# tingliu/glia

Hardware: AMD Instinct MI355X
Metric: region_merges_per_sec (higher is better)
Workload: dtype u32 labels / f32 image / f64 statistics and features

## Files before the change

### cli/edge_rebuild_check.cpp

```cpp
#include <cstdio>
#include <cstring>
#include <vector>
#include "../glia_amd/csrc/edge_record.hpp"

using namespace glia;

int main() {
  const uint32_t R = 5, R0 = 1;
  struct E { uint32_t u, v, n; double mean; uint32_t r0; bool h0; };
  const std::vector<E> edges = {{0, 1, 7, 0.125, 1, true},  {0, 2, 3, 0.5, 0, true},       {1, 2, 11, 0.33203125, 0, false}, {1, 3, 1, 0.0, 2, true},
                                {2, 3, 40, 0.99609375, 1, false}, {0, 4, 5, 0.25, 3, true}, {2, 4, 9, 0.7421875, 2, true},    {3, 4, 2, 0.00390625, 1, true}};
  std::vector<uint32_t> deg(R, 0), off(R, 0), cur(R, 0);
  for (const E& e : edges) { ++deg[e.u]; ++deg[e.v]; }
  for (uint32_t r = 1; r < R; ++r) off[r] = off[r - 1] + deg[r - 1];
  std::vector<FatEntry> pool(2 * edges.size());
  std::vector<uint32_t> posu(edges.size()), posv(edges.size());
  for (size_t e = 0; e < edges.size(); ++e) {
    const E& g = edges[e];
    const uint32_t pu = cur[g.u]++, pv = cur[g.v]++;
    FatEntry a; a.eid = (uint32_t)e; a.rs = g.v; a.n = g.n; a.pos = pv; a.off = off[g.v]; a.len = deg[g.v]; a.mean = g.mean;
    FatEntry b = a; b.rs = g.u; b.pos = pu; b.off = off[g.u]; b.len = deg[g.u];
    pool[off[g.u] + pu] = a; pool[off[g.v] + pv] = b;
    posu[e] = pu; posv[e] = pv;
  }
  int checked = 0, cats[3] = {0, 0, 0};
  for (uint32_t v = 0; v < R; ++v) {
    for (uint32_t i = 0; i < deg[v]; ++i) {
      const FatEntry& fe = pool[off[v] + i];
      if (fe.eid == kRecNone || !(fe.rs < v)) continue;
      const E& g = edges[fe.eid];
      const uint32_t rs = g.u, r2 = g.v, k = r2 - R0;
      const uint32_t cat = rs < g.r0 ? 0u : (g.h0 ? 1u : 2u);
      const unsigned long long seq = ((unsigned long long)(k + 1u) << 32) | ((unsigned long long)cat << 30) | rs;
      const double first = g.mean, sal = -first;
      unsigned long long mb, sb;
      memcpy(&mb, &first, 8); memcpy(&sb, &sal, 8);
      const uint32_t want[16] = {rs, r2, posu[fe.eid], posv[fe.eid], (uint32_t)mb, (uint32_t)(mb >> 32), g.n, kRecNone,
                                 off[rs], deg[rs], off[r2], deg[r2], (uint32_t)sb, (uint32_t)(sb >> 32), (uint32_t)seq, (uint32_t)(seq >> 32)};
      const EdgeRec got = rebuild_edge_record(fe, i, v, off[v], deg[v], (uint32_t)((seq >> 30) & 3u), R0);
      if (memcmp(&got, want, 64) != 0) {
        const uint32_t* w = reinterpret_cast<const uint32_t*>(&got);
        printf("edge_rebuild_check: edge %u (%u, %u) differs:", fe.eid, rs, r2);
        for (int j = 0; j < 16; ++j) printf(" %08x/%08x", w[j], want[j]);
        printf("\n");
        return 1;
      }
      ++checked; ++cats[cat];
    }
  }
  if (checked != (int)edges.size() || !cats[0] || !cats[1] || !cats[2]) { printf("edge_rebuild_check: %d of %zu edges visited\n", checked, edges.size()); return 1; }
  printf("edge_rebuild_check: %d records rebuilt from list entries agree with the stored form (cat 0/1/2: %d/%d/%d)\n", checked, cats[0], cats[1], cats[2]);
  return 0;
}
```

### glia_amd/csrc/api.cpp

```cpp
#include <algorithm>
#include <atomic>
#include <cmath>
#include <cstdlib>
#include <cstring>
#include <limits>
#include <mutex>
#include <unordered_map>

#include "rmap_order.hpp"
#include "api_types.hpp"

namespace glia {

static thread_local std::string g_err;
void set_error(const std::string& msg) { g_err = msg; }

static const char* const kOptionKeys[] = {"GLIA_HMT_PB_WINDOW", "GLIA_HMT_PB_BATCH", "GLIA_HMT_WINCAP", "GLIA_HMT_REBASE", "GLIA_HMT_HORIZON",
                                          "GLIA_HMT_FORCE_TREE", "GLIA_HMT_HELPERS", "GLIA_HMT_TRACE", "GLIA_HMT_LIBM", "GLIA_HMT_BC_NOCOMMON",
                                          "GLIA_HMT_BC_GENERIC", "GLIA_HMT_DEBUG", "GLIA_HMT_MAXITERS", "GLIA_HMT_MINCAP", "GLIA_HMT_MEDIAN_BATCH", "GLIA_HMT_BCFEAT", "GLIA_HMT_CC"};
static std::mutex g_opt_mu;
static std::unordered_map<std::string, std::string> g_opt;
static bool g_opt_init = false;
static void opt_init_locked() {
  if (g_opt_init) return;
  for (const char* k : kOptionKeys) if (const char* e = getenv(k)) g_opt[k] = e;
  g_opt_init = true;
}
static bool opt_known(const char* key) { for (const char* k : kOptionKeys) if (!strcmp(k, key)) return true; return false; }
bool option(const char* key, std::string* value) {
  std::lock_guard<std::mutex> lock(g_opt_mu);
  opt_init_locked();
  auto it = g_opt.find(key);
  if (it == g_opt.end()) return false;
  if (value) *value = it->second;
  return true;
}
int set_option(const char* key, const char* value) {
  if (!key || !opt_known(key)) { set_error(std::string("set_option: unknown option ") + (key ? key : "(null)")); return GLIA_HMT_ERR_ARG; }
  std::lock_guard<std::mutex> lock(g_opt_mu);
  opt_init_locked();
  if (value) g_opt[key] = value; else g_opt.erase(key);
  return GLIA_HMT_OK;
}

float ceil_f32(double d) {
  if (std::isinf(d) || std::isnan(d)) return (float)d;
  float f = (float)d;
  if ((double)f < d) f = std::nextafterf(f, std::numeric_limits<float>::infinity());
  return f;
}
static float floor_f32(double d) {
  if (std::isinf(d) || std::isnan(d)) return (float)d;
  float f = (float)d;
  if ((double)f > d) f = std::nextafterf(f, -std::numeric_limits<float>::infinity());
  return f;
}
uint32_t next_pow2(uint64_t v) {
  uint64_t p = 1;
  while (p < v) p <<= 1;
  return (uint32_t)std::min<uint64_t>(p, 1ull << 31);
}

HistSpec make_hist_spec(int bins, double lo, double hi) {
  HistSpec h;
  h.bins = bins;
  double interval = (hi - lo) / bins;
  double b = 0.0;
  for (int i = 0; i < GLIA_HMT_MAX_BINS; ++i) {
    if (i < bins) { b = (i == 0) ? interval : b + interval; h.fb[i] = ceil_f32(b); }
    else h.fb[i] = std::numeric_limits<float>::infinity();
  }
  h.lo_f = floor_f32(lo);
  h.hi_f = ceil_f32(hi);
  return h;
}

static LibmSel probe_host_libm() {
  std::vector<double> xs;
  uint64_t s = 0x9E3779B97F4A7C15ull;
  auto next = [&]() { s ^= s << 13; s ^= s >> 7; s ^= s << 17; return s; };
  for (int i = 0; i < 6000; ++i) { const uint64_t n = 1 + next() % 100000, c = 1 + next() % n; xs.push_back((double)c / (double)n); }
  for (int i = 0; i < 3000; ++i) xs.push_back(1.0 + ((double)(int64_t)(next() % 2000001) - 1000000.0) * 1e-7);
  for (int i = 0; i < 3000; ++i) xs.push_back(std::ldexp(1.0 + (double)(next() >> 12) * 0x1p-52, (int)(next() % 120) - 60));
  for (int e = -1074; e < 1024; e += 37) xs.push_back(std::ldexp(1.0, e));
  LibmSel sel = {kLibmDevice, kLibmDevice, kLibmDevice};
  bool l2 = true, ls = true, lf = true, ps = true, pf = true;
  for (double x : xs) {
    volatile double vx = x;
    const double h2 = std::log2(vx), h1 = std::log(vx);
    l2 = l2 && glibc::as_u64(h2) == glibc::as_u64(glibc::log2_sse2(x));
    ls = ls && glibc::as_u64(h1) == glibc::as_u64(glibc::log_sse2(x));
    lf = lf && glibc::as_u64(h1) == glibc::as_u64(glibc::log_fma(x));
  }
  for (int i = 0; i < 12000; ++i) {
    const double x = i < 4000 ? (double)(i + 1) : (double)(1 + next() % (i < 8000 ? (1ull << 24) : (1ull << 40)));
    volatile double vx = x, vy = 1.5;
    const uint64_t h = glibc::as_u64(std::pow(vx, vy));
    ps = ps && h == glibc::as_u64(glibc::pow_sse2(x, 1.5));
    pf = pf && h == glibc::as_u64(glibc::pow_fma(x, 1.5));
  }
  if (l2) sel.log2_variant = kLibmSse2;
  if (lf) sel.log_variant = kLibmFma; else if (ls) sel.log_variant = kLibmSse2;
  if (pf) sel.pow_variant = kLibmFma; else if (ps) sel.pow_variant = kLibmSse2;
  std::string ov;
  if (option("GLIA_HMT_LIBM", &ov)) {
    const char* e = ov.c_str();
    const int v = !strcmp(e, "sse2") ? kLibmSse2 : !strcmp(e, "fma") ? kLibmFma : kLibmDevice;
    sel.log_variant = v; sel.log2_variant = v == kLibmFma ? kLibmSse2 : v; sel.pow_variant = v;
  }
  return sel;
}

}

static std::atomic<int> g_live_contexts{0};

extern "C" {

const char* glia_hmt_last_error(void) { return g_err.c_str(); }
const char* glia_hmt_version(void) { return "glia_hmt 0.1 (gfx950)"; }

int glia_hmt_ctx_create(int device, void* hip_stream, glia_hmt_ctx** out) {
  if (!out) { set_error("ctx_create: out is NULL"); return GLIA_HMT_ERR_ARG; }
  int n = 0;
  GLIA_HIP_TRY(hipGetDeviceCount(&n));
  if (device < 0 || device >= n) { set_error("ctx_create: no such HIP device"); return GLIA_HMT_ERR_ARG; }
  GLIA_HIP_TRY(hipSetDevice(device));
  glia_hmt_ctx* c = new glia_hmt_ctx;
  c->device = device;
  ++g_live_contexts;
  const int rc = [&]() -> int {
    if (hip_stream) c->stream = (hipStream_t)hip_stream;
    else { GLIA_HIP_TRY(hipStreamCreateWithFlags(&c->stream, hipStreamNonBlocking)); c->own_stream = true; }
    GLIA_HIP_TRY(hipMalloc(&c->flags, 256));
    GLIA_HIP_TRY(hipMemsetAsync(c->flags, 0, 256, c->stream));
    GLIA_HIP_TRY(hipEventCreate(&c->ev0));
    GLIA_HIP_TRY(hipEventCreate(&c->ev1));
    return GLIA_HMT_OK;
  }();
  if (rc) { glia_hmt_ctx_destroy(c); return rc; }
  static const LibmSel sel = probe_host_libm();
  c->libm = sel;
  *out = c;
  if (sel.log2_variant == 0 || sel.log_variant == 0 || sel.pow_variant == 0)
    set_error(std::string("warning: the host libm's ") + (sel.log2_variant == 0 ? "log2 " : "") + (sel.log_variant == 0 ? "log " : "") +
              (sel.pow_variant == 0 ? "pow " : "") + "is not reproduced bit for bit by a restatement (glibc 2.35 FMA / non-FMA builds): "
              "the entropy / log / compactness feature columns are within 1 ulp of this host's values, unpinned; equal classifier scores may order differently");
  return GLIA_HMT_OK;
}

int glia_hmt_ctx_libm(const glia_hmt_ctx* c, int* log2_variant, int* log_variant) {
  if (!c) return GLIA_HMT_ERR_ARG;
  if (log2_variant) *log2_variant = c->libm.log2_variant;
  if (log_variant) *log_variant = c->libm.log_variant;
  return GLIA_HMT_OK;
}

int glia_hmt_ctx_libm_status(const glia_hmt_ctx* c) {
  if (!c) return GLIA_HMT_ERR_ARG;
  return (c->libm.log2_variant != 0 && c->libm.log_variant != 0 && c->libm.pow_variant != 0) ? 1 : 0;
}

int glia_hmt_ctx_libm_pow(const glia_hmt_ctx* c, int* pow_variant) {
  if (!c || !pow_variant) return GLIA_HMT_ERR_ARG;
  *pow_variant = c->libm.pow_variant;
  return GLIA_HMT_OK;
}

int glia_hmt_host_libm_probe_pow(int* pow_variant) {
  if (!pow_variant) return GLIA_HMT_ERR_ARG;
  *pow_variant = probe_host_libm().pow_variant;
  return GLIA_HMT_OK;
}

int glia_hmt_host_rmap_ranks(const uint32_t* labels, const int64_t* first_voxel, int64_t n, int mode, uint32_t* rank) {
  if (!labels || !first_voxel || !rank || n < 0 || mode < 0 || mode > 2) { set_error("host_rmap_ranks: invalid argument"); return GLIA_HMT_ERR_ARG; }
  std::vector<uint32_t> lab(labels, labels + n), out;
  std::vector<long long> first(first_voxel, first_voxel + n);
  for (int64_t i = 1; i < n; ++i) if (lab[i] <= lab[i - 1]) { set_error("host_rmap_ranks: labels must be ascending"); return GLIA_HMT_ERR_ARG; }
  rmap_ranks(lab, first, &out, mode);
  std::copy(out.begin(), out.end(), rank);
  return GLIA_HMT_OK;
}

int glia_hmt_host_libm_probe(int* log2_variant, int* log_variant) {
  const LibmSel sel = probe_host_libm();
  if (log2_variant) *log2_variant = sel.log2_variant;
  if (log_variant) *log_variant = sel.log_variant;
  return GLIA_HMT_OK;
}

int glia_hmt_host_libm_eval(int function, int variant, const double* h_in, double* h_out, int64_t n) {
  if (!h_in || !h_out || n < 0 || function < 0 || function > 2 || (variant != kLibmSse2 && variant != kLibmFma)) {
    set_error("host_libm_eval: invalid argument");
    return GLIA_HMT_ERR_ARG;
  }
  for (int64_t i = 0; i < n; ++i) {
    const double x = h_in[i];
    if (function == 2) h_out[i] = !glibc::pow_in_domain(x, 1.5) ? std::pow(x, 1.5) : variant == kLibmFma ? glibc::pow_fma(x, 1.5) : glibc::pow_sse2(x, 1.5);
    else h_out[i] = function == 0 ? glibc::log2_sse2(x) : variant == kLibmFma ? glibc::log_fma(x) : glibc::log_sse2(x);
  }
  return GLIA_HMT_OK;
}

int glia_hmt_libm_eval(glia_hmt_ctx* c, int function, int variant, const double* d_in, double* d_out, int64_t n) {
  if (!c || !d_in || !d_out || n < 0 || function < 0 || function > 2) { set_error("libm_eval: invalid argument"); return GLIA_HMT_ERR_ARG; }
  GLIA_HIP_TRY(hipSetDevice(c->device));
  return launch_libm_eval(function, variant, d_in, d_out, n, c->stream);
}

unsigned long long glia_hmt_release_cached_memory(void) { return (unsigned long long)glia::BlockCache::get().trim(); }
unsigned long long glia_hmt_internal_errors(void) { return glia::internal_errors(); }
int glia_hmt_set_option(const char* key, const char* value) { return glia::set_option(key, value); }
int glia_hmt_check_merge_order(const uint32_t* h_order, int64_t n_merges, int64_t n_regions, int64_t* first_bad) {
  if ((!h_order && n_merges) || n_merges < 0 || n_regions < 0 || n_regions > 0x7FFFFFFFll) { set_error("check_merge_order: invalid argument"); return GLIA_HMT_ERR_ARG; }
  int64_t bad = -1;
  if (glia::merge_order_is_consistent(h_order, n_merges, (uint32_t)n_regions, &bad)) { if (first_bad) *first_bad = -1; return GLIA_HMT_OK; }
  if (first_bad) *first_bad = bad;
  set_error("check_merge_order: merge " + std::to_string(bad) + " joins a region that does not exist (any more) or creates the wrong one");
  return GLIA_HMT_ERR_ARG;
}

void glia_hmt_ctx_destroy(glia_hmt_ctx* c) {
  if (!c) return;
  (void)hipSetDevice(c->device);
  if (c->stream) (void)hipStreamSynchronize(c->stream);
  (void)free_tables(c);
  if (c->flags) (void)hipFree(c->flags);
  if (c->ev0) (void)hipEventDestroy(c->ev0);
  if (c->ev1) (void)hipEventDestroy(c->ev1);
  if (c->own_stream) (void)hipStreamDestroy(c->stream);
  delete c;
  if (--g_live_contexts <= 0) (void)glia::BlockCache::get().trim();
}

int glia_hmt_ctx_sync(glia_hmt_ctx* c) {
  if (!c) return GLIA_HMT_ERR_ARG;
  GLIA_HIP_TRY(hipStreamSynchronize(c->stream));
  return GLIA_HMT_OK;
}

int glia_hmt_ctx_set_table_hint(glia_hmt_ctx* c, int64_t expected_regions, int64_t expected_pairs) {
  if (!c) return GLIA_HMT_ERR_ARG;
  c->hint_rcap = expected_regions > 0 ? next_pow2((uint64_t)expected_regions * 2) : 0;
  c->hint_pcap = expected_pairs > 0 ? next_pow2((uint64_t)expected_pairs * 2) : 0;
  return GLIA_HMT_OK;
}

int glia_hmt_synth(glia_hmt_ctx* c, int dim, const int64_t dims[3], int S, int G, uint64_t seed, int variant,
                   uint32_t* d_labels, float* d_pb) {
  if (!c || !dims || !d_labels || !d_pb || (dim != 2 && dim != 3) || S <= 0 || G <= 0) {
    set_error("synth: invalid argument");
    return GLIA_HMT_ERR_ARG;
  }
  GLIA_HIP_TRY(hipSetDevice(c->device));
  int64_t N = dims[0] * dims[1] * (dim == 3 ? dims[2] : 1);
  OwnedArrays own;
  uint32_t* d_truth = nullptr;
  int rc = own.alloc(&d_truth, (size_t)N);
  if (rc == GLIA_HMT_OK) rc = launch_synth(dim, dims, S, G, seed, variant, d_labels, d_truth, d_pb, c->stream);
  if (rc == GLIA_HMT_OK) GLIA_HIP_TRY(hipStreamSynchronize(c->stream));
  return rc;
}

int glia_hmt_watershed(glia_hmt_ctx* c, int dim, const int64_t dims[3], const float* d_image, double level, uint32_t* d_labels, uint32_t* n_labels,
                       int* sweeps) {
  if (!c || !dims || !d_image || !d_labels || (dim != 2 && dim != 3) || !(level >= 0.0)) { set_error("watershed: invalid argument"); return GLIA_HMT_ERR_ARG; }
  GLIA_HIP_TRY(hipSetDevice(c->device));
  return watershed_labels(dim, dims, d_image, level, d_labels, n_labels, sweeps, c->stream);
}

int glia_hmt_label_components(glia_hmt_ctx* c, int dim, const int64_t dims[3], const uint32_t* d_labels_in, const uint32_t* d_mask, int mode,
                              uint32_t* d_labels_out, uint32_t* n_components) {
  auto bad = [](const char* what) { set_error(std::string("label_components: ") + what); return GLIA_HMT_ERR_ARG; };
  if (!c || !dims || !d_labels_in || !d_labels_out || !n_components) return bad("ctx, dims, the two volumes and n_components must not be NULL");
  if (dim != 2 && dim != 3) return bad("dim must be 2 or 3");
  const uint64_t most = 0xFFFFFFFEull;
  uint64_t n = 1;
  for (int i = 0; i < dim; ++i) {
    if (dims[i] <= 0) return bad("extents must be positive");
    if ((uint64_t)dims[i] > most / n) return bad("between 1 and 2^32 - 2 voxels");
    n *= (uint64_t)dims[i];
  }
  if (mode < GLIA_HMT_CC_IDENTITY || mode > GLIA_HMT_CC_BINARY_INVERTED) return bad("mode must be 0 (identity), 1 (binary) or 2 (binary, inverted)");
  if (d_labels_out == d_labels_in) return bad("the volume cannot be labelled in place");
  int route = GLIA_HMT_CC_ROUTE_TILED;
  std::string v;
  if (option("GLIA_HMT_CC", &v) && v != "tiled") {
    if (v != "global") return bad(("GLIA_HMT_CC must be tiled or global, not '" + v + "'").c_str());
    route = GLIA_HMT_CC_ROUTE_GLOBAL;
  }
  GLIA_HIP_TRY(hipSetDevice(c->device));
  return label_components(dim, dims, d_labels_in, d_mask, mode, route, d_labels_out, n_components, c->stream);
}

static int overlap_args(const char* who, const glia_hmt_ctx* c, const uint32_t* d_a, const uint32_t* d_b, int64_t n_voxels) {
  auto bad = [&](const char* what) { set_error(std::string(who) + ": " + what); return GLIA_HMT_ERR_ARG; };
  if (!c) return bad("ctx must not be NULL");
  if (!d_a || !d_b) return bad("the two label volumes must not be NULL");
  if (n_voxels < 1 || (uint64_t)n_voxels > 0xFFFFFFFEull) return bad("between 1 and 2^32 - 2 voxels");
  return GLIA_HMT_OK;
}

int glia_hmt_label_overlap(glia_hmt_ctx* c, const uint32_t* d_a, const uint32_t* d_b, const uint32_t* d_mask, int64_t n_voxels, int flags,
                           glia_hmt_overlap_entry* h_entries, int64_t capacity, int64_t* n_entries) {
  auto bad = [](const char* what) { set_error(std::string("label_overlap: ") + what); return GLIA_HMT_ERR_ARG; };
  if (int rc = overlap_args("label_overlap", c, d_a, d_b, n_voxels)) return rc;
  if (!n_entries) return bad("n_entries must not be NULL");
  if (capacity < 0 || (capacity > 0 && !h_entries)) return bad("h_entries must hold `capacity` >= 0 entries");
  if (flags & ~(GLIA_HMT_OVERLAP_DROP_ZERO_A | GLIA_HMT_OVERLAP_DROP_ZERO_B)) return bad("unknown flag bits");
  GLIA_HIP_TRY(hipSetDevice(c->device));
  std::vector<glia_hmt_overlap_entry> table;
  OverlapPass pass;
  if (int rc = label_overlap(d_a, d_b, d_mask, (unsigned long long)n_voxels, flags, c->stream, &table, &pass)) return rc;
  c->evt = glia_hmt_eval_timing{pass.ms, (int64_t)table.size(), pass.repeats};
  *n_entries = (int64_t)table.size();
  if ((int64_t)table.size() > capacity) { set_error("label_overlap: " + std::to_string(table.size()) + " entries, capacity " + std::to_string(capacity)); return GLIA_HMT_ERR_CAPACITY; }
  std::copy(table.begin(), table.end(), h_entries);
  return GLIA_HMT_OK;
}

int glia_hmt_eval(glia_hmt_ctx* c, int n_images, const uint32_t* const* d_res, const uint32_t* const* d_ref, const uint32_t* const* d_mask,
                  const int64_t* n_voxels, int vi_mode, glia_hmt_eval_result* out) {
  auto bad = [](const char* what) { set_error(std::string("eval: ") + what); return GLIA_HMT_ERR_ARG; };
  if (!c) return bad("ctx must not be NULL");
  if (n_images < 1) return bad("at least one image pair");
  if (!d_res || !d_ref || !n_voxels || !out) return bad("d_res, d_ref, n_voxels and out must not be NULL");
  if (vi_mode != GLIA_HMT_VI_REFERENCE && vi_mode != GLIA_HMT_VI_EXACT) return bad("vi_mode must be GLIA_HMT_VI_REFERENCE or GLIA_HMT_VI_EXACT");
  for (int i = 0; i < n_images; ++i) if (int rc = overlap_args("eval", c, d_res[i], d_ref[i], n_voxels[i])) return rc;
  GLIA_HIP_TRY(hipSetDevice(c->device));
  std::vector<std::vector<glia_hmt_overlap_entry>> tables((size_t)n_images);
  std::vector<const glia_hmt_overlap_entry*> ptr((size_t)n_images);
  std::vector<int64_t> len((size_t)n_images);
  glia_hmt_eval_timing t = {0, 0, 0};
  for (int i = 0; i < n_images; ++i) {
    OverlapPass pass;
    if (int rc = label_overlap(d_res[i], d_ref[i], d_mask ? d_mask[i] : nullptr, (unsigned long long)n_voxels[i], GLIA_HMT_OVERLAP_DROP_ZERO_B, c->stream,
                               &tables[i], &pass)) return rc;
    t.ms_count += pass.ms; t.entries += (int64_t)tables[i].size(); t.repeats += pass.repeats;
    ptr[i] = tables[i].data(); len[i] = (int64_t)tables[i].size();
  }
  c->evt = t;
  return overlap_scores(ptr.data(), len.data(), n_images, vi_mode, out);
}

int glia_hmt_last_eval_timing(const glia_hmt_ctx* c, glia_hmt_eval_timing* out) {
  if (!c || !out) { set_error("last_eval_timing: invalid argument"); return GLIA_HMT_ERR_ARG; }
  *out = c->evt;
  return GLIA_HMT_OK;
}

int64_t glia_hmt_transform_keys(const uint32_t* h_order, int64_t n_merges, uint32_t* h_src, uint32_t* h_dst, int64_t capacity) {
  if (!h_order || !h_src || !h_dst || n_merges < 0) { set_error("transform_keys: invalid argument"); return GLIA_HMT_ERR_ARG; }
  std::vector<uint32_t> s, d;
  int rc = transform_keys(h_order, n_merges, &s, &d);
  if (rc) return rc;
  if ((int64_t)s.size() > capacity) { set_error("transform_keys: output capacity too small"); return GLIA_HMT_ERR_CAPACITY; }
  std::copy(s.begin(), s.end(), h_src);
  std::copy(d.begin(), d.end(), h_dst);
  return (int64_t)s.size();
}

int glia_hmt_transform_image(glia_hmt_ctx* c, uint32_t* d_labels, int64_t n_voxels, const uint32_t* h_src, const uint32_t* h_dst,
                             int64_t n_map, const uint32_t* d_mask, int fill_missing) {
  if (!c || !d_labels || n_voxels < 0 || n_map < 0 || (n_map && (!h_src || !h_dst))) { set_error("transform_image: invalid argument"); return GLIA_HMT_ERR_ARG; }
  GLIA_HIP_TRY(hipSetDevice(c->device));
  return transform_image(d_labels, n_voxels, h_src, h_dst, n_map, d_mask, fill_missing, c->stream, &c->transform_ms);
}

int glia_hmt_relabel_image(glia_hmt_ctx* c, uint32_t* d_labels, int64_t n_voxels, int64_t min_size, uint32_t* n_labels) {
  if (!c || !d_labels || n_voxels < 0 || !n_labels) { set_error("relabel_image: invalid argument"); return GLIA_HMT_ERR_ARG; }
  GLIA_HIP_TRY(hipSetDevice(c->device));
  return relabel_image(d_labels, n_voxels, min_size, n_labels, c->stream);
}

double glia_hmt_last_transform_ms(const glia_hmt_ctx* c) { return c ? c->transform_ms : 0.0; }

int64_t glia_hmt_gen_tree(const uint32_t* h_order, int64_t n_merges, uint32_t* node_label, int32_t* parent, int32_t* child0,
                          int32_t* child1, int64_t capacity) {
  if (!h_order || !node_label || !parent || !child0 || !child1 || n_merges < 0) { set_error("gen_tree: invalid argument"); return GLIA_HMT_ERR_ARG; }
  return gen_tree(h_order, n_merges, node_label, parent, child0, child1, capacity);
}

}
```

### glia_amd/csrc/edge_record.hpp

```cpp
#pragma once
#include <stdint.h>

#if defined(__HIPCC__)
#define GLIA_REC_HD __host__ __device__
#else
#define GLIA_REC_HD
#endif

namespace glia {

#if defined(__HIPCC__)
typedef uint2 RecPair;
#else
struct RecPair { uint32_t x, y; };
#endif
constexpr uint32_t kRecNone = 0xFFFFFFFFu;

struct __attribute__((aligned(16))) FatEntry {
  uint32_t eid;
  uint32_t rs;
  uint32_t n;
  uint32_t pos;
  uint32_t off;
  uint32_t len;
  double mean;
};
static_assert(sizeof(FatEntry) == 32, "FatEntry layout");

struct __attribute__((aligned(16))) EdgeRec {
  uint32_t u, v, posu, posv;
  double mean; int n; uint32_t next;
  RecPair hu, hv;
  double sal; unsigned long long seq;
};
static_assert(sizeof(EdgeRec) == 64, "EdgeRec layout");

GLIA_REC_HD inline EdgeRec rebuild_edge_record(const FatEntry& fe, uint32_t idx, uint32_t v, uint32_t voff, uint32_t vlen, uint32_t cat, uint32_t R0) {
  EdgeRec r;
  r.u = fe.rs; r.v = v; r.posu = fe.pos; r.posv = idx;
  r.mean = fe.mean; r.n = (int)fe.n; r.next = kRecNone;
  r.hu.x = fe.off; r.hu.y = fe.len; r.hv.x = voff; r.hv.y = vlen;
  r.sal = -fe.mean;
  r.seq = ((unsigned long long)(v - R0 + 1u) << 32) | ((unsigned long long)(cat & 3u) << 30) | fe.rs;
  return r;
}

}
```

### glia_amd/csrc/greedy.hip

```cpp
#include <atomic>
#include <cstring>
#include <vector>
#include <limits>
#include <rocprim/device/device_scan.hpp>
#include <rocprim/device/device_radix_sort.hpp>
#include <rocprim/device/device_segmented_radix_sort.hpp>

#include "greedy_batch.hpp"

namespace glia {

__global__ void pq_build_level_kernel(PqTree t, int l) {
  const int lane = threadIdx.x & 63;
  uint32_t j = (blockIdx.x * blockDim.x + threadIdx.x) >> 6;
  if (j < t.lv[l].size) (void)pq_recompute_node(t, l, j, lane, true);
}

int pq_setup(DeviceBuffers& buf, PqTree& t, hipStream_t stream) {
  t.nlevels = 0;
  uint32_t n = t.nleaves;
  while (true) {
    n = (n + kFan - 1) / kFan;
    if (t.nlevels >= kMaxLevels) { set_error("greedy: edge table too large"); return GLIA_HMT_ERR_ARG; }
    PqLevel& L = t.lv[t.nlevels++];
    L.size = n;
    int rc;
    if ((rc = buf.get(&L.sal, n, false, stream))) return rc;
    if ((rc = buf.get(&L.seq, n, false, stream))) return rc;
    if ((rc = buf.get(&L.arg, n, false, stream))) return rc;
    if ((rc = buf.get(&L.dirty, n, true, stream))) return rc;
    if (n <= kTopMax) break;
  }
  {
    int rc;
    if ((rc = buf.get(&t.glist[0], t.lv[0].size, false, stream))) return rc;
    if ((rc = buf.get(&t.glist[1], t.lv[0].size, false, stream))) return rc;
    if ((rc = buf.get(&t.gcount, 2, true, stream))) return rc;
  }
  for (int l = 0; l < t.nlevels; ++l) {
    unsigned long long threads = (unsigned long long)t.lv[l].size * 64ull;
    hipLaunchKernelGGL(pq_build_level_kernel, dim3((unsigned)((threads + 255) / 256)), dim3(256), 0, stream, t, l);
  }
  GLIA_HIP_TRY(hipGetLastError());
  return GLIA_HMT_OK;
}

namespace {

__global__ void win_range_kernel(const double* sal, uint32_t E0, unsigned long long* mm) {
  unsigned long long lo = ~0ull, hi = 0ull;
  for (uint32_t i = blockIdx.x * blockDim.x + threadIdx.x; i < E0; i += gridDim.x * blockDim.x) {
    const unsigned long long b = f64_ord(sal[i]);
    lo = b < lo ? b : lo; hi = b > hi ? b : hi;
  }
  atomicMin(&mm[0], lo); atomicMax(&mm[1], hi);
}
__global__ void win_params_kernel(const unsigned long long* mm, uint32_t B, double* range) {
  const double smin = f64_unord(mm[0]), smax = f64_unord(mm[1]);
  range[0] = smin;
  range[1] = smax > smin ? (double)B / (smax - smin) : 0.0;
}
__global__ void win_collect_kernel(const EdgeRec* er, uint32_t n_edges, const uint8_t* rdead, unsigned long long* kseq, uint32_t* vals, uint32_t* counter) {
  const uint32_t e = blockIdx.x * blockDim.x + threadIdx.x;
  if (e >= n_edges) return;
  const unsigned long long q = er[e].seq;
  if (q == 0) return;
  const uint2 uv = *reinterpret_cast<const uint2*>(&er[e].u);
  if (rdead[uv.x] | rdead[uv.y]) return;
  const uint32_t i = atomicAdd(counter, 1u);
  kseq[i] = q; vals[i] = e;
}
__global__ void win_collect_lists_kernel(WinState st, uint32_t n_regions, unsigned long long* kseq, uint32_t* vals, uint32_t cap, uint32_t* counter) {
  const uint32_t r = (blockIdx.x * blockDim.x + threadIdx.x) >> 6, lane = threadIdx.x & 63u;
  if (r >= n_regions || st.rdead[r]) return;
  const uint32_t off = st.adj_off[r], len = st.adj_len[r];
  const double smin = st.wrange[0], scale = st.wrange[1];
  uint32_t rebuilt = 0;
  for (uint32_t base = 0; base < len; base += 64u) {
    const uint32_t i = base + lane;
    unsigned long long q = 0;
    uint32_t e = kNone;
    if (i < len) {
      const FatEntry fe = st.fpool[off + i];
      if (fe.eid != kNone && fe.rs < r && !st.rdead[fe.rs]) {
        e = fe.eid;
        if ((unsigned long long)e >= st.ne_base && win_cell(-fe.mean, smin, scale, st.wB) < st.wch) {
          const EdgeRec rec = rebuild_edge_record(fe, i, r, off, len, st.ecat[e], st.R0);
          st.er[e] = rec;
          q = rec.seq; ++rebuilt;
        } else q = st.er[e].seq;
      }
    }
    const unsigned long long m = __ballot(q != 0);
    if (m == 0) continue;
    const int first = (int)__builtin_ctzll(m);
    uint32_t b0 = 0;
    if ((int)lane == first) b0 = atomicAdd(&counter[0], (uint32_t)__popcll(m));
    b0 = (uint32_t)__shfl((int)b0, first);
    const uint32_t o = b0 + (uint32_t)__popcll(m & ((1ull << lane) - 1ull));
    if (q != 0 && o < cap) { kseq[o] = q; vals[o] = e; }
  }
  if (rebuilt) atomicAdd(&counter[1], rebuilt);
}
__global__ void win_salkey_kernel(const EdgeRec* er, const uint32_t* vals, uint32_t n, unsigned long long* ksal) {
  const uint32_t i = blockIdx.x * blockDim.x + threadIdx.x;
  if (i < n) ksal[i] = f64_ord(er[vals[i]].sal);
}
__global__ void win_baseline_fill_kernel(WinState st, uint32_t n, uint32_t* isort_w, unsigned long long* isort_seq) {
  const uint32_t i = blockIdx.x * blockDim.x + threadIdx.x;
  if (i >= n) return;
  const EdgeRec r = st.er[isort_w[i]];
  isort_seq[i] = r.seq;
  atomicAdd(&st.wcnt[win_cell(r.sal, st.wrange[0], st.wrange[1], st.wB)], 1u);
}
__global__ void win_segments_kernel(WinState st, const uint32_t* isort, uint32_t n, uint32_t* ige) {
  const uint32_t c = blockIdx.x * blockDim.x + threadIdx.x;
  if (c > st.wB) return;
  uint32_t lo = 0, hi = n;
  while (lo < hi) {
    const uint32_t mid = (lo + hi) >> 1;
    if (win_cell(st.er[isort[mid]].sal, st.wrange[0], st.wrange[1], st.wB) >= c) lo = mid + 1; else hi = mid;
  }
  ige[c] = c == 0 ? n : lo;
}
__global__ void adj_fill_fat(GreedyState g, WinState st, uint32_t E0, uint32_t* cursor) {
  const uint32_t e = blockIdx.x * blockDim.x + threadIdx.x;
  if (e >= E0) return;
  const uint32_t u = g.e_u[e], v = g.e_v[e];
  const uint32_t pu = atomicAdd(&cursor[u], 1u), pv = atomicAdd(&cursor[v], 1u);
  const uint32_t ou = g.adj_off[u], ov = g.adj_off[v], lu = g.adj_len[u], lv = g.adj_len[v];
  FatEntry a; a.eid = e; a.rs = v; a.n = (uint32_t)g.e_n[e]; a.pos = pv; a.off = ov; a.len = lv; a.mean = g.e_mean[e];
  FatEntry b = a; b.rs = u; b.pos = pu; b.off = ou; b.len = lu;
  st.fpool[ou + pu] = a; g.e_posu[e] = pu;
  st.fpool[ov + pv] = b; g.e_posv[e] = pv;
  EdgeRec r; r.u = u; r.v = v; r.posu = pu; r.posv = pv; r.mean = g.e_mean[e]; r.n = g.e_n[e]; r.next = kNone;
  r.hu = make_uint2(ou, lu); r.hv = make_uint2(ov, lv); r.sal = g.pq.leaf_sal[e]; r.seq = g.pq.leaf_seq[e];
  st.er[e] = r;
}
__global__ void fat_to_thin(const FatEntry* f, uint2* out, unsigned long long n) {
  const unsigned long long i = (unsigned long long)blockIdx.x * blockDim.x + threadIdx.x;
  if (i < n) { const FatEntry fe = f[i]; out[i] = make_uint2(fe.eid, fe.eid == kNone ? 0u : fe.rs); }
}
__global__ void edge_unpack(GreedyState g, const EdgeRec* er, const uint8_t* rdead, uint32_t n) {
  const uint32_t e = blockIdx.x * blockDim.x + threadIdx.x;
  if (e >= n) return;
  const EdgeRec r = er[e];
  g.e_u[e] = r.u; g.e_v[e] = r.v; g.e_posu[e] = r.posu; g.e_posv[e] = r.posv; g.e_mean[e] = r.mean; g.e_n[e] = r.n;
  g.pq.leaf_sal[e] = r.sal; g.pq.leaf_seq[e] = (rdead[r.u] | rdead[r.v]) ? 0ull : r.seq;
}

__global__ void edge_unpack_live(GreedyState g, const EdgeRec* er, const uint32_t* vals, uint32_t n) {
  const uint32_t i = blockIdx.x * blockDim.x + threadIdx.x;
  if (i >= n) return;
  const uint32_t e = vals[i];
  const EdgeRec r = er[e];
  g.e_u[e] = r.u; g.e_v[e] = r.v; g.e_posu[e] = r.posu; g.e_posv[e] = r.posv; g.e_mean[e] = r.mean; g.e_n[e] = r.n;
  g.pq.leaf_sal[e] = r.sal; g.pq.leaf_seq[e] = r.seq;
}

__global__ void edge_flags(const uint32_t* pa, const uint32_t* pb, long long P, uint32_t* flag, long long* partner) {
  long long i = (long long)blockIdx.x * blockDim.x + threadIdx.x;
  if (i >= P) return;
  uint32_t a = pa[i], b = pb[i];
  long long j = (a < b) ? find_pair(pa, pb, P, b, a) : -1;
  flag[i] = j >= 0 ? 1u : 0u;
  partner[i] = j;
}

__global__ void edge_fill(const uint32_t* pa, const uint32_t* pb, const uint32_t* prec, long long P,
                          const uint32_t* flag, const uint32_t* eidx, const long long* partner,
                          const uint32_t* rlabel, uint32_t R, GreedyState st, uint32_t* deg) {
  long long i = (long long)blockIdx.x * blockDim.x + threadIdx.x;
  if (i >= P || !flag[i]) return;
  const uint32_t e = eidx[i];
  const long long j = partner[i];
  const uint32_t u = find_label(rlabel, R, pa[i]), v = find_label(rlabel, R, pb[i]);
  const uint32_t* wi = &prec[(size_t)i * kPairWords];
  const uint32_t* wj = &prec[(size_t)j * kPairWords];
  double si, sj;
  memcpy(&si, &wi[P_SUM], 8);
  memcpy(&sj, &wj[P_SUM], 8);
  const int n = (int)(wi[P_CNT] + wj[P_CNT]);
  const double mean = sdivide(si + sj, (double)n, 0.0);
  st.e_u[e] = u; st.e_v[e] = v; st.e_mean[e] = mean; st.e_n[e] = n;
  st.pq.leaf_sal[e] = -mean; st.pq.leaf_seq[e] = (unsigned long long)e + 1ull;
  atomicAdd(&deg[u], 1u);
  atomicAdd(&deg[v], 1u);
}

__global__ void adj_fill(GreedyState st, uint32_t E0, uint32_t* cursor) {
  uint32_t e = blockIdx.x * blockDim.x + threadIdx.x;
  if (e >= E0) return;
  const uint32_t u = st.e_u[e], v = st.e_v[e];
  const uint32_t pu = atomicAdd(&cursor[u], 1u), pv = atomicAdd(&cursor[v], 1u);
  st.pool[st.adj_off[u] + pu] = make_uint2(e, v); st.e_posu[e] = pu;
  st.pool[st.adj_off[v] + pv] = make_uint2(e, u); st.e_posv[e] = pv;
}

__global__ void region_sizes(const uint32_t* rrec, uint32_t R, unsigned long long* rsz, double* rsum) {
  uint32_t r = blockIdx.x * blockDim.x + threadIdx.x;
  if (r >= R) return;
  const uint32_t* w = &rrec[(size_t)r * kRegionWords];
  rsz[r] = w[R_CNT];
  double d; memcpy(&d, &w[R_SUM], 8); rsum[r] = d;
}

__global__ void median_collect(VolumeRef vol, const uint32_t* pa, const uint32_t* pb, long long P, const uint32_t* flag,
                               const uint32_t* eidx, const unsigned long long* e_off, uint32_t* cursor, float* out) {
  const long long N = vol.nx * vol.ny * vol.nz;
  const long long p = (long long)blockIdx.x * blockDim.x + threadIdx.x;
  if (p >= N) return;
  const long long x = p % vol.nx, y = (p / vol.nx) % vol.ny, z = p / (vol.nx * vol.ny);
  const uint32_t t = vol.lab[p];
  if (t == kMaskedLabel) return;
  uint32_t nb = t;
  const long long sy = vol.nx, sz = vol.nx * vol.ny;
  const uint32_t* L = vol.lab_nb;
  do {
    uint32_t q;
    if (x > 0 && (q = L[p - 1]) != t && q != kMaskedLabel) { nb = q; break; }
    if (x + 1 < vol.nx && (q = L[p + 1]) != t && q != kMaskedLabel) { nb = q; break; }
    if (y > 0 && (q = L[p - sy]) != t && q != kMaskedLabel) { nb = q; break; }
    if (y + 1 < vol.ny && (q = L[p + sy]) != t && q != kMaskedLabel) { nb = q; break; }
    if (vol.dim == 3) {
      if (z > 0 && (q = L[p - sz]) != t && q != kMaskedLabel) { nb = q; break; }
      if (z + 1 < vol.nz && (q = L[p + sz]) != t && q != kMaskedLabel) { nb = q; break; }
    }
  } while (false);
  if (nb == t) return;
  const long long i = find_pair(pa, pb, P, t < nb ? t : nb, t < nb ? nb : t);
  if (i < 0 || !flag[i]) return;
  const uint32_t e = eidx[i];
  out[e_off[e] + atomicAdd(&cursor[e], 1u)] = vol.pb[p];
}

__global__ void median_from_runs(const unsigned long long* pv_off, const float* pv, unsigned long long nV, const uint32_t* pa, const uint32_t* pb, long long P,
                                 const uint32_t* flag, const uint32_t* eidx, const unsigned long long* e_off, float* out) {
  const unsigned long long v = (unsigned long long)blockIdx.x * blockDim.x + threadIdx.x;
  if (v >= nV) return;
  long long lo = 0, hi = P;
  while (lo < hi) { const long long mid = (lo + hi) >> 1; if (pv_off[mid + 1] <= v) lo = mid + 1; else hi = mid; }
  const long long i = lo;
  const uint32_t a = pa[i], b = pb[i];
  const long long owner = a < b ? i : find_pair(pa, pb, P, b, a);
  if (owner < 0 || !flag[owner]) return;
  const unsigned long long first = owner == i ? 0ull : pv_off[owner + 1] - pv_off[owner];
  out[e_off[eidx[owner]] + first + (v - pv_off[i])] = pv[v];
}

__global__ void median_init(GreedyState st, uint32_t E0) {
  const uint32_t e = blockIdx.x * blockDim.x + threadIdx.x;
  if (e >= E0) return;
  const uint32_t n = (uint32_t)st.e_n[e];
  const double med = (double)st.vals[st.e_off[e] + n / 2u];
  st.e_mean[e] = med;
  st.pq.leaf_sal[e] = st.size_weight ? -med * (double)min(st.rsz[st.e_u[e]], st.rsz[st.e_v[e]]) : -med;
  atomicAdd(&st.rbv[st.e_u[e]], (unsigned long long)n);
  atomicAdd(&st.rbv[st.e_v[e]], (unsigned long long)n);
}

__global__ void fill_leaves_dead(PqTree t, uint32_t from) {
  uint32_t i = from + blockIdx.x * blockDim.x + threadIdx.x;
  if (i < t.nleaves) { t.leaf_seq[i] = 0; t.leaf_sal[i] = -__builtin_inf(); }
}

}

struct WinBaseline {
  unsigned long long *kseq = nullptr, *kseq2 = nullptr, *ksal = nullptr, *ksal2 = nullptr, *iseq = nullptr;
  uint32_t *vals = nullptr, *vals2 = nullptr, *isort = nullptr, *ige = nullptr, *counter = nullptr;
  void* tmp = nullptr; size_t tmp_bytes = 0;
  uint32_t E0 = 0;
  double h_range[2] = {0.0, 0.0};
  long long prev_top_cell = -1;
  unsigned long long prev_ne = 0;
  double horizon_factor = 0.0;
  bool from_lists = false;
  unsigned long long rebuilt_last = 0;

  int init(DeviceBuffers& buf, WinState& ws, const double* leaf_sal, uint32_t n_initial, uint32_t B, uint32_t R, hipStream_t stream) {
    int rc;
    E0 = n_initial;
    unsigned long long* mm; double* range;
    if ((rc = buf.get(&ws.rdead, 2 * (size_t)R, true, stream))) return rc;
    if ((rc = buf.get(&ws.whead, B, false, stream))) return rc;
    if ((rc = buf.get(&ws.wcnt, B, true, stream))) return rc;
    if ((rc = buf.get(&isort, E0, false, stream))) return rc;
    if ((rc = buf.get(&iseq, E0, false, stream))) return rc;
    if ((rc = buf.get(&ige, (size_t)B + 1, false, stream))) return rc;
    if ((rc = buf.get(&mm, 2, false, stream))) return rc;
    if ((rc = buf.get(&range, 2, false, stream))) return rc;
    if ((rc = buf.get(&kseq, E0, false, stream))) return rc;
    if ((rc = buf.get(&kseq2, E0, false, stream))) return rc;
    if ((rc = buf.get(&ksal, E0, false, stream))) return rc;
    if ((rc = buf.get(&ksal2, E0, false, stream))) return rc;
    if ((rc = buf.get(&vals, E0, false, stream))) return rc;
    if ((rc = buf.get(&vals2, E0, false, stream))) return rc;
    if ((rc = buf.get(&counter, 2, true, stream))) return rc;
    GLIA_HIP_TRY(rocprim::radix_sort_pairs_desc(nullptr, tmp_bytes, kseq, kseq2, vals, vals2, (size_t)E0, 0, 64, stream));
    if ((rc = buf.get((char**)&tmp, tmp_bytes ? tmp_bytes : 16, false, stream))) return rc;
    ws.wrange = range; ws.isort = isort; ws.isort_seq = iseq; ws.ige = ige;
    const unsigned long long mm0[2] = {~0ull, 0ull};
    GLIA_HIP_TRY(hipMemcpyAsync(mm, mm0, sizeof(mm0), hipMemcpyHostToDevice, stream));
    hipLaunchKernelGGL(win_range_kernel, dim3(256), dim3(256), 0, stream, leaf_sal, E0, mm);
    hipLaunchKernelGGL(win_params_kernel, dim3(1), dim3(1), 0, stream, mm, B, range);
    GLIA_HIP_TRY(hipGetLastError());
    GLIA_HIP_TRY(hipMemcpyAsync(h_range, range, sizeof(h_range), hipMemcpyDeviceToHost, stream));
    GLIA_HIP_TRY(hipStreamSynchronize(stream));
    return GLIA_HMT_OK;
  }
  int collect(const WinState& ws, uint32_t n_edges, uint32_t n_regions, hipStream_t stream, uint32_t* n_out) {
    GLIA_HIP_TRY(hipMemsetAsync(counter, 0, 2 * sizeof(uint32_t), stream));
    if (from_lists) hipLaunchKernelGGL(win_collect_lists_kernel, dim3((unsigned)(((unsigned long long)n_regions * 64ull + 255ull) / 256ull)), dim3(256), 0, stream, ws, n_regions, kseq, vals, E0, counter);
    else hipLaunchKernelGGL(win_collect_kernel, dim3((n_edges + 255) / 256), dim3(256), 0, stream, ws.er, n_edges, ws.rdead, kseq, vals, counter);
    GLIA_HIP_TRY(hipGetLastError());
    uint32_t h[2] = {0, 0};
    GLIA_HIP_TRY(hipMemcpyAsync(h, counter, sizeof(h), hipMemcpyDeviceToHost, stream));
    GLIA_HIP_TRY(hipStreamSynchronize(stream));
    if (h[0] > E0) { set_error("greedy: more live edges than initial edges (internal error)"); return GLIA_HMT_ERR_INTERNAL; }
    *n_out = h[0]; rebuilt_last = h[1];
    return GLIA_HMT_OK;
  }
  int rebaseline(WinState& ws, uint32_t n_edges, unsigned long long* ctrl, hipStream_t stream) {
    uint32_t n = 0;
    if (int rc = collect(ws, n_edges, ws.R0 + (uint32_t)ctrl[CTRL_MERGES], stream, &n)) return rc;
    if (n) {
      size_t bytes = tmp_bytes;
      GLIA_HIP_TRY(rocprim::radix_sort_pairs_desc(tmp, bytes, kseq, kseq2, vals, vals2, (size_t)n, 0, 64, stream));
      hipLaunchKernelGGL(win_salkey_kernel, dim3((n + 255) / 256), dim3(256), 0, stream, ws.er, vals2, n, ksal);
      bytes = tmp_bytes;
      GLIA_HIP_TRY(rocprim::radix_sort_pairs_desc(tmp, bytes, ksal, ksal2, vals2, isort, (size_t)n, 0, 64, stream));
    }
    GLIA_HIP_TRY(hipMemsetAsync(ws.whead, 0xFF, sizeof(uint32_t) * ws.wB, stream));
    GLIA_HIP_TRY(hipMemsetAsync(ws.wcnt, 0, sizeof(uint32_t) * ws.wB, stream));
    if (n) hipLaunchKernelGGL(win_baseline_fill_kernel, dim3((n + 255) / 256), dim3(256), 0, stream, ws, n, isort, iseq);
    hipLaunchKernelGGL(win_segments_kernel, dim3((ws.wB + 1 + 255) / 256), dim3(256), 0, stream, ws, isort, n, ige);
    GLIA_HIP_TRY(hipGetLastError());
    ws.nsort = n;
    std::string renv;
    ws.rebase_after = option("GLIA_HMT_REBASE", &renv) ? strtoull(renv.c_str(), nullptr, 10) : std::max<unsigned long long>(800000ull, (unsigned long long)n / 2ull);
    ws.wch = 0;
    if (horizon_factor > 0.0 && n > 4096) {
      unsigned long long topkey = 0;
      GLIA_HIP_TRY(hipMemcpyAsync(&topkey, ksal2, sizeof(topkey), hipMemcpyDeviceToHost, stream));
      GLIA_HIP_TRY(hipStreamSynchronize(stream));
      const long long top_cell = (long long)win_cell(f64_unord(topkey), h_range[0], h_range[1], ws.wB);
      if (prev_top_cell >= 0 && n_edges > prev_ne) {
        const double d = (double)std::max<long long>(0, prev_top_cell - top_cell);
        const double delta = std::max(horizon_factor * d * (double)ws.rebase_after / (double)(n_edges - prev_ne), (double)ws.wB / 512.0);
        ws.wch = (double)top_cell > delta ? (uint32_t)((double)top_cell - delta) : 0u;
      }
      prev_top_cell = top_cell; prev_ne = n_edges;
    }
    ws.ne_base = n_edges;
    const double inf = std::numeric_limits<double>::infinity();
    ctrl[CTRL_CTHR] = (unsigned long long)(long long)(ws.wB - 1);
    memcpy(&ctrl[CTRL_TSAL], &inf, 8); ctrl[CTRL_TSEQ] = ~0ull; ctrl[CTRL_IPTR] = 0;
    return GLIA_HMT_OK;
  }
};

static int run_pb_loop(const RagArrays& rag, hipStream_t stream, const PbRequest& req, MergeResult* out) {
  const long long P = rag.P;
  const uint32_t R = (uint32_t)rag.R;
  if (R == 0 || P == 0) return GLIA_HMT_OK;
  const VolumeRef* median_of = req.median_of;
  CallEvents<3> ev;
  int rc;
  if ((rc = ev.create())) return rc;
  GLIA_HIP_TRY(hipEventRecord(ev.ev[0], stream));
  DeviceBuffers buf;
  uint32_t* flag; uint32_t* eidx; long long* partner;
  if ((rc = buf.get(&flag, P + 1, true, stream))) return rc;
  if ((rc = buf.get(&eidx, P + 1, false, stream))) return rc;
  if ((rc = buf.get(&partner, P, false, stream))) return rc;
  hipLaunchKernelGGL(edge_flags, dim3((unsigned)((P + 255) / 256)), dim3(256), 0, stream, rag.d_pa, rag.d_pb, P, flag, partner);
  if ((rc = rocprim_run(buf, stream, [&](void* t, size_t& b) {
        return rocprim::exclusive_scan(t, b, flag, eidx, 0u, (size_t)(P + 1), rocprim::plus<uint32_t>(), stream); }))) return rc;
  uint32_t E0 = 0;
  GLIA_HIP_TRY(hipMemcpyAsync(&E0, eidx + P, sizeof(uint32_t), hipMemcpyDeviceToHost, stream));
  GLIA_HIP_TRY(hipStreamSynchronize(stream));
  if (E0 == 0) return GLIA_HMT_OK;

  GreedyState st;
  memset(&st, 0, sizeof(st));
  st.R0 = R;
  const bool mincap = initial_capacities(E0, 18, 36, &st.Ecap, &st.pool_cap);
  if ((rc = buf.get(&st.adj_off, 2 * (size_t)R, true, stream))) return rc;
  if ((rc = buf.get(&st.adj_len, 2 * (size_t)R + 1, true, stream))) return rc;
  std::string o_window, o_batch, o_txt;
  const bool batch_off = option("GLIA_HMT_PB_BATCH", &o_batch) && o_batch[0] == '0';
  bool window = !median_of && !req.size_weight && !(option("GLIA_HMT_PB_WINDOW", &o_window) && o_window[0] == '0');
  WinState ws;
  memset(&ws, 0, sizeof(ws));
  GrowList edges, entries, values;
  if (window) {
    if ((rc = entries.add(buf, &ws.fpool, st.pool_cap, stream))) return rc;
    if ((rc = edges.add(buf, &ws.er, st.Ecap, stream))) return rc;
    if ((rc = edges.add(buf, &ws.ecat, st.Ecap, stream))) return rc;
  }
  else if ((rc = entries.add(buf, &st.pool, st.pool_cap, stream))) return rc;
  if ((rc = edges.add(buf, &st.e_u, st.Ecap, stream)) || (rc = edges.add(buf, &st.e_v, st.Ecap, stream)) ||
      (rc = edges.add(buf, &st.e_posu, st.Ecap, stream)) || (rc = edges.add(buf, &st.e_posv, st.Ecap, stream)) ||
      (rc = edges.add(buf, &st.e_mean, st.Ecap, stream)) || (rc = edges.add(buf, &st.e_n, st.Ecap, stream, true)) ||
      (rc = edges.add(buf, &st.pq.leaf_sal, st.Ecap, stream)) || (rc = edges.add(buf, &st.pq.leaf_seq, st.Ecap, stream)))
    return rc;
  st.pq.nleaves = st.Ecap;
  if ((rc = buf.get(&st.rsz, 2 * (size_t)R, true, stream))) return rc;
  if ((rc = buf.get(&st.rsum, 2 * (size_t)R, true, stream))) return rc;
  st.cond_n = req.cond_n; st.cond_rpb = req.cond_rpb; st.size_weight = req.size_weight ? 1 : 0;
  st.cond_t0 = req.cond_n > 0 ? (unsigned long long)req.cond_sizes[0] : 0; st.cond_t1 = req.cond_n > 1 ? (unsigned long long)req.cond_sizes[1] : 0;
  hipLaunchKernelGGL(region_sizes, dim3((R + 255) / 256), dim3(256), 0, stream, rag.d_rrec, R, st.rsz, st.rsum);
  if ((rc = buf.get(&st.mark0, 2 * (size_t)R, true, stream))) return rc;
  if ((rc = buf.get(&st.mark1, 2 * (size_t)R, true, stream))) return rc;
  if ((rc = buf.get(&st.order, 3 * ((size_t)R + 16), false, stream))) return rc;
  if ((rc = buf.get(&st.sal_out, (size_t)R + 16, false, stream))) return rc;
  if ((rc = buf.get(&st.ctrl, 16, true, stream))) return rc;
  uint32_t* cursor;
  if ((rc = buf.get(&cursor, 2 * (size_t)R, true, stream))) return rc;

  hipLaunchKernelGGL(fill_leaves_dead, dim3((st.Ecap - E0 + 255) / 256), dim3(256), 0, stream, st.pq, E0);
  hipLaunchKernelGGL(edge_fill, dim3((unsigned)((P + 255) / 256)), dim3(256), 0, stream, rag.d_pa, rag.d_pb, rag.d_prec, P,
                     flag, eidx, partner, rag.d_rlabel, R, st, st.adj_len);
  if ((rc = rocprim_run(buf, stream, [&](void* t, size_t& b) {
        return rocprim::exclusive_scan(t, b, st.adj_len, st.adj_off, 0u, (size_t)R, rocprim::plus<uint32_t>(), stream); }))) return rc;
  if (window) hipLaunchKernelGGL(adj_fill_fat, dim3((E0 + 255) / 256), dim3(256), 0, stream, st, ws, E0, cursor);
  else hipLaunchKernelGGL(adj_fill, dim3((E0 + 255) / 256), dim3(256), 0, stream, st, E0, cursor);
  GLIA_HIP_TRY(hipGetLastError());
  unsigned long long n_values = 0;
  if (median_of) {
    if ((rc = edges.add(buf, &st.e_off, st.Ecap, stream))) return rc;
    if ((rc = buf.get(&st.rbv, 2 * (size_t)R, true, stream))) return rc;
    if ((rc = rocprim_run(buf, stream, [&](void* t, size_t& b) {
          return rocprim::exclusive_scan(t, b, st.e_n, st.e_off, 0ull, (size_t)E0 + 1, rocprim::plus<unsigned long long>(), stream); }))) return rc;
    GLIA_HIP_TRY(hipMemcpyAsync(&n_values, st.e_off + E0, sizeof(n_values), hipMemcpyDeviceToHost, stream));
    GLIA_HIP_TRY(hipStreamSynchronize(stream));
    if (n_values >= 0xFFFFFFFFull) { set_error("merge_order_pb: more than 2^32 boundary voxels (median linkage)"); return GLIA_HMT_ERR_ARG; }
    st.vals_cap = mincap ? std::max(n_values, 1ull) : n_values * 4ull + (1ull << 20);
    float* unsorted;
    if ((rc = values.add(buf, &st.vals, (size_t)st.vals_cap, stream))) return rc;
    if ((rc = buf.get(&unsorted, (size_t)n_values, false, stream))) return rc;
    uint32_t* vcursor;
    if ((rc = buf.get(&vcursor, (size_t)E0, true, stream))) return rc;
    if (median_of->lab) {
      const long long N = median_of->nx * median_of->ny * median_of->nz;
      hipLaunchKernelGGL(median_collect, dim3((unsigned)((N + 255) / 256)), dim3(256), 0, stream, *median_of, rag.d_pa, rag.d_pb, P,
                         flag, eidx, st.e_off, vcursor, unsorted);
    } else {
      if (!rag.d_pv_off) { set_error("merge_order_pb: median linkage needs the volume or the map's boundary values"); return GLIA_HMT_ERR_UNSUPPORTED; }
      if (rag.nV) hipLaunchKernelGGL(median_from_runs, dim3((unsigned)((rag.nV + 255) / 256)), dim3(256), 0, stream, rag.d_pv_off, rag.d_pv, rag.nV, rag.d_pa, rag.d_pb,
                                     (long long)P, flag, eidx, st.e_off, unsorted);
    }
    GLIA_HIP_TRY(hipGetLastError());
    if ((rc = rocprim_run(buf, stream, [&](void* t, size_t& b) {
          return rocprim::segmented_radix_sort_keys(t, b, unsorted, st.vals, (unsigned)n_values, (unsigned)E0, st.e_off, st.e_off + 1, 0, 32, stream); }))) return rc;
    hipLaunchKernelGGL(median_init, dim3((E0 + 255) / 256), dim3(256), 0, stream, st, E0);
    GLIA_HIP_TRY(hipGetLastError());
  }
  unsigned long long ctrl[CTRL_WORDS] = {};
  ctrl[CTRL_EDGES] = E0; ctrl[CTRL_ENTRIES] = 2ull * E0; ctrl[CTRL_STATUS] = ST_RUN; ctrl[CTRL_VALUES] = n_values;
  WinBaseline base;
  if (window) {
    uint32_t B = 256;
    while (B < E0 / 4 && B < (1u << 22)) B <<= 1;
    ws.wB = B; ws.R0 = R;
    ws.wcap = kWinCap; ws.wbudget = kWinBudget;
    ws.force_tree = 0;
    if (option("GLIA_HMT_FORCE_TREE", &o_txt)) ws.force_tree = strtoull(o_txt.c_str(), nullptr, 10);
    if (option("GLIA_HMT_WINCAP", &o_txt)) {
      const uint32_t c = (uint32_t)strtoul(o_txt.c_str(), nullptr, 10);
      if (c >= 16 && c <= kWinCap) { ws.wcap = c; ws.wbudget = c / 2; }
    }
    ws.order = st.order; ws.sal_out = st.sal_out; ws.ctrl = st.ctrl; ws.rsz = st.rsz; ws.rsum = st.rsum;
    ws.mark0 = st.mark0; ws.mark1 = st.mark1; ws.adj_off = st.adj_off; ws.adj_len = st.adj_len;
    ws.pool_cap = st.pool_cap; ws.Ecap = st.Ecap;
    ws.cond_n = st.cond_n; ws.cond_t0 = st.cond_t0; ws.cond_t1 = st.cond_t1; ws.cond_rpb = st.cond_rpb;
    if ((rc = base.init(buf, ws, st.pq.leaf_sal, E0, B, R, stream))) return rc;
    if (req.cond_n <= 0 && !batch_off) base.horizon_factor = option("GLIA_HMT_HORIZON", &o_txt) ? atof(o_txt.c_str()) : 0.5;
    base.from_lists = req.cond_n <= 0 && !batch_off;
    if ((rc = base.rebaseline(ws, E0, ctrl, stream))) return rc;
  } else if ((rc = pq_setup(buf, st.pq, stream))) return rc;
  GLIA_HIP_TRY(hipMemcpyAsync(st.ctrl, ctrl, sizeof(ctrl), hipMemcpyHostToDevice, stream));
  GLIA_HIP_TRY(hipEventRecord(ev.ev[1], stream));


  st.max_iters = window ? 1ull << 22 : 1ull << 16;
  const bool trace = option("GLIA_HMT_TRACE");
  if (option("GLIA_HMT_MAXITERS", &o_txt)) st.max_iters = std::max(1ull, strtoull(o_txt.c_str(), nullptr, 10));
  const auto kernel = [&]() { return !window ? "tree" : req.cond_n > 0 ? "window" : "batch"; };
  const auto unhandled = [&]() {
    set_error(std::string("greedy: the ") + kernel() + " kernel stopped with status " + std::to_string(ctrl[CTRL_STATUS]) + ", which its driver does not handle (internal error)");
    return GLIA_HMT_ERR_INTERNAL;
  };
  while (true) {
    if (window) {
      ws.max_iters = st.max_iters;
      if (req.cond_n > 0) hipLaunchKernelGGL(greedy_window_kernel<true>, dim3(1), dim3(kGreedyThreads), 0, stream, ws);
      else if (batch_off) hipLaunchKernelGGL(greedy_window_kernel<false>, dim3(1), dim3(kGreedyThreads), 0, stream, ws);
      else hipLaunchKernelGGL(greedy_batch_kernel, dim3(1), dim3(kGreedyThreads), 0, stream, ws);
    } else if (median_of) hipLaunchKernelGGL(greedy_pb_kernel<true>, dim3(1), dim3(kGreedyThreads), 0, stream, st);
    else hipLaunchKernelGGL(greedy_pb_kernel<false>, dim3(1), dim3(kGreedyThreads), 0, stream, st);
    GLIA_HIP_TRY(hipGetLastError());
    GLIA_HIP_TRY(hipMemcpyAsync(ctrl, st.ctrl, sizeof(ctrl), hipMemcpyDeviceToHost, stream));
    GLIA_HIP_TRY(hipStreamSynchronize(stream));
    if (trace) fprintf(stderr, "[trace] merge loop launch ended: status %llu, merges %llu of %u regions, edges %llu, list entries %llu, records rebuilt %llu\n", ctrl[CTRL_STATUS], ctrl[CTRL_MERGES], R, ctrl[CTRL_EDGES], ctrl[CTRL_ENTRIES], base.rebuilt_last);
    base.rebuilt_last = 0;
    if (ctrl[CTRL_STATUS] == ST_DONE) break;
    switch (ctrl[CTRL_STATUS]) {
      case ST_RUN:
        if (!window) continue;
        break;
      case ST_REBASE:
        if (!window) return unhandled();
        break;
      case ST_BAD_SALIENCY: set_error("Error: invalid boundary saliency..."); return GLIA_HMT_ERR_SALIENCY;
      case ST_INTERNAL: {
        char msg[256];
        snprintf(msg, sizeof(msg), "greedy: window queue overflow or more merges than regions (internal error: merges %llu of %u regions, %llu edges of %u initial, "
                 "window %llu%s, %s kernel)", ctrl[CTRL_MERGES], R, ctrl[CTRL_EDGES], E0, ctrl[CTRL_WFILL], ctrl[CTRL_WERR] ? " overflowed" : "", kernel());
        set_error(msg);
        return GLIA_HMT_ERR_INTERNAL;
      }
      case ST_NEED_TREE:
        if (!window) return unhandled();
        entries.remove(&ws.fpool);
        edges.remove(&ws.er);
        edges.remove(&ws.ecat);
        if ((rc = entries.add(buf, &st.pool, st.pool_cap, stream))) return rc;
        hipLaunchKernelGGL(fat_to_thin, dim3((unsigned)((ctrl[CTRL_ENTRIES] + 255) / 256)), dim3(256), 0, stream, ws.fpool, st.pool, ctrl[CTRL_ENTRIES]);
        if (base.from_lists) {
          uint32_t n_live = 0;
          if ((rc = base.collect(ws, (uint32_t)ctrl[CTRL_EDGES], R + (uint32_t)ctrl[CTRL_MERGES], stream, &n_live))) return rc;
          hipLaunchKernelGGL(fill_leaves_dead, dim3((st.Ecap + 255) / 256), dim3(256), 0, stream, st.pq, 0u);
          if (n_live) hipLaunchKernelGGL(edge_unpack_live, dim3((n_live + 255) / 256), dim3(256), 0, stream, st, ws.er, base.vals, n_live);
        } else
        hipLaunchKernelGGL(edge_unpack, dim3((unsigned)((ctrl[CTRL_EDGES] + 255) / 256)), dim3(256), 0, stream, st, ws.er, ws.rdead, (uint32_t)ctrl[CTRL_EDGES]);
        GLIA_HIP_TRY(hipGetLastError());
        if ((rc = pq_setup(buf, st.pq, stream))) return rc;
        window = false;
        st.max_iters = 1ull << 16;
        break;
      case ST_NEED_POOL: {
        const unsigned long long ncap = st.pool_cap * 2;
        if ((rc = entries.grow(buf, (size_t)st.pool_cap, (size_t)ncap, stream))) return rc;
        st.pool_cap = ncap; ws.pool_cap = ncap;
        break;
      }
      case ST_NEED_VALUES: {
        if (!median_of) return unhandled();
        const unsigned long long ncap = st.vals_cap * 2;
        if ((rc = values.grow(buf, (size_t)ctrl[CTRL_VALUES], (size_t)ncap, stream))) return rc;
        st.vals_cap = ncap;
        break;
      }
      case ST_NEED_EDGES: {
        if (st.Ecap >= kMaxEdgeSlots) { set_error("greedy: more than 2^32 edge slots needed"); return GLIA_HMT_ERR_ARG; }
        const uint32_t ocap = st.Ecap, ncap = (uint32_t)std::min<unsigned long long>(kMaxEdgeSlots, (unsigned long long)ocap * 2ull);
        if ((rc = edges.grow(buf, ocap, ncap, stream))) return rc;
        st.Ecap = ncap; st.pq.nleaves = ncap; ws.Ecap = ncap;
        hipLaunchKernelGGL(fill_leaves_dead, dim3((ncap - ocap + 255) / 256), dim3(256), 0, stream, st.pq, ocap);
        if (!window && (rc = pq_setup(buf, st.pq, stream))) return rc;
        break;
      }
      default: return unhandled();
    }
    if (window) {
      if ((rc = base.rebaseline(ws, (uint32_t)ctrl[CTRL_EDGES], ctrl, stream))) return rc;
      GLIA_HIP_TRY(hipMemcpyAsync(st.ctrl + CTRL_CTHR, ctrl + CTRL_CTHR, 4 * sizeof(unsigned long long), hipMemcpyHostToDevice, stream));
    }
    unsigned long long zero = ST_RUN;
    GLIA_HIP_TRY(hipMemcpyAsync(st.ctrl + CTRL_STATUS, &zero, sizeof(zero), hipMemcpyHostToDevice, stream));
  }
  GLIA_HIP_TRY(hipEventRecord(ev.ev[2], stream));
  GLIA_HIP_TRY(hipEventSynchronize(ev.ev[2]));
  out->ms_table = ev.ms(0, 1); out->ms_loop = ev.ms(1, 2);
  out->n_scored = (int64_t)ctrl[CTRL_EDGES];
  return copy_merges(out, (int64_t)ctrl[CTRL_MERGES], st.order, st.sal_out);
}


static std::atomic<unsigned long long> g_internal_errors{0};
unsigned long long internal_errors() { return g_internal_errors.load(); }
void count_internal_error() { g_internal_errors.fetch_add(1); }
bool merge_order_is_consistent(const uint32_t* o, int64_t n, uint32_t R, int64_t* first_bad) {
  std::vector<uint8_t> gone(2 * (size_t)R + 1, 0);
  for (int64_t k = 0; k < n; ++k) {
    const uint32_t a = o[3 * k], b = o[3 * k + 1], c = o[3 * k + 2];
    if (k >= (int64_t)R || c != R + (uint32_t)k || a >= c || b >= c || a == b || gone[a] || gone[b]) { if (first_bad) *first_bad = k; return false; }
    gone[a] = gone[b] = 1;
  }
  return true;
}
int finish_merge_order(int rc, const uint32_t* o, int64_t n, uint32_t R, hipStream_t stream) {
  int64_t bad = -1;
  if (rc == GLIA_HMT_OK && !merge_order_is_consistent(o, n, R, &bad)) {
    set_error("greedy: merge " + std::to_string(bad) + " of " + std::to_string(n) + " joins a region that does not exist (any more) or creates the wrong one (internal error)");
    rc = GLIA_HMT_ERR_INTERNAL;
  }
  if (rc == GLIA_HMT_ERR_INTERNAL) { count_internal_error(); (void)hipStreamSynchronize(stream); }
  return rc;
}
int greedy_mean(const RagArrays& rag, hipStream_t stream, const PbRequest& req, MergeResult* out) {
  const int rc = run_pb_loop(rag, stream, req, out);
  return finish_merge_order(rc, out->order.data(), out->n, (uint32_t)rag.R, stream);
}

}
```

### glia_amd/csrc/greedy_batch.hpp

```cpp
#pragma once
#include "greedy_window.hpp"

namespace glia {
namespace {

constexpr uint32_t kBatchKill = 32;
constexpr int kMemP = 3;
constexpr uint32_t kMemMax = 192;
struct BatchShared {
  alignas(16) Key part1[kNW];
  alignas(16) Key part2[kNW];
  uint32_t nkill, kovf; alignas(16) uint32_t kill[kBatchKill];
  uint32_t byrank[kNW];
  uint32_t bitmap[kNW][64];
  uint32_t m_newcount[kNW], m_total[kNW], m_ok[kNW];
  double m_maxsal[kNW];
  uint32_t bad;
};

template <int CTRL, int ROW_MASK = 0xf>
__device__ __forceinline__ void top2_ord_step(unsigned long long& a1, unsigned long long& a2) {
  const unsigned long long b1 = dpp64<CTRL, ROW_MASK, ROW_MASK != 0xf>(a1), b2 = dpp64<CTRL, ROW_MASK, ROW_MASK != 0xf>(a2);
  const bool g = b1 > a1;
  const unsigned long long hi = g ? b1 : a1, lo = g ? a1 : b1, m2 = b2 > a2 ? b2 : a2;
  a1 = hi; a2 = lo > m2 ? lo : m2;
}
__device__ __forceinline__ void wave_top2_ord(unsigned long long& a1, unsigned long long& a2) {
  top2_ord_step<0xB1>(a1, a2);
  top2_ord_step<0x4E>(a1, a2);
  top2_ord_step<0x124>(a1, a2);
  top2_ord_step<0x128>(a1, a2);
  top2_ord_step<0x142, 0xa>(a1, a2);
  top2_ord_step<0x143, 0xc>(a1, a2);
  a1 = lane_u64(a1, 63); a2 = lane_u64(a2, 63);
}

#ifdef GLIA_HMT_PROFILE
__device__ unsigned long long g_scanprof[8];
__device__ unsigned long long g_scanfill[3][3];
#define SCAN_T(i) do { if (tid == 0) { const unsigned long long tn_ = __builtin_readcyclecounter(); g_scanprof[i] += tn_ - st_; st_ = tn_; } } while (0)
#else
#define SCAN_T(i) do {} while (0)
#endif
enum { kScanOther = 0, kScanNarrow = 1, kScanWide = 2 };
__device__ __forceinline__ void batch_scan(const WinState& st, WinShared& w, BatchShared& b, int tid, [[maybe_unused]] int from) {
#ifdef GLIA_HMT_PROFILE
  unsigned long long st_ = __builtin_readcyclecounter();
  if (tid == 0) g_scanprof[7] += 1;
#endif
  const uint32_t n = w.n < st.wcap ? w.n : st.wcap, nk = b.nkill < kBatchKill ? b.nkill : kBatchKill, kovf = b.kovf;
#ifdef GLIA_HMT_PROFILE
  if (tid == 0) g_scanfill[from][n <= 512u ? 0 : n <= 1024u ? 1 : 2] += 1;
#endif
  const uint32_t own = 64u * (uint32_t)(((tid >> 6) + (tid & 63)) & 7) + (uint32_t)(tid & 63);
  Key k1, k2;
  k1.sal = -__builtin_inf(); k1.seq = 0; k1.arg = 0; k2 = k1;
  auto pass = [&](auto nb_tag) {
    constexpr int NB = decltype(nb_tag)::value;
    unsigned long long q[NB]; uint32_t e[NB]; double sl[NB];
#pragma unroll
    for (int j = 0; j < NB; ++j) { const uint32_t i = own + (uint32_t)j * kGreedyThreads; q[j] = w.seq[i]; e[j] = w.e[i]; sl[j] = w.sal[i]; }
    const uint4 ka = *reinterpret_cast<const uint4*>(&b.kill[0]), kb = *reinterpret_cast<const uint4*>(&b.kill[4]);
    const uint32_t kl[8] = {ka.x, ka.y, ka.z, ka.w, kb.x, kb.y, kb.z, kb.w};
    SCAN_T(0);
    uint32_t deadm[NB];
#pragma unroll
    for (int j = 0; j < NB; ++j) {
      uint32_t d = 0;
#pragma unroll
      for (uint32_t t = 0; t < 8; ++t) d |= (uint32_t)(t < nk) & (uint32_t)(kl[t] == e[j]);
      deadm[j] = d;
    }
    if (nk > 8u) {
      for (uint32_t t = 8; t < nk; ++t) {
        const uint32_t kt = b.kill[t];
#pragma unroll
        for (int j = 0; j < NB; ++j) deadm[j] |= (uint32_t)(kt == e[j]);
      }
      if (kovf) {
        full_barrier();
#pragma unroll
        for (int j = 0; j < NB; ++j) {
          const uint32_t i = own + (uint32_t)j * kGreedyThreads;
          if (i < n && q[j] != 0) deadm[j] |= (uint32_t)(st.er[e[j]].seq == 0);
        }
      }
    }
#pragma unroll
    for (int j = 0; j < NB; ++j) {
      const uint32_t i = own + (uint32_t)j * kGreedyThreads;
      const bool was = (i < n) & (q[j] != 0);
      const bool live = was & (deadm[j] == 0u);
      if (was & !live) w.seq[i] = 0;
      Key c; c.sal = live ? sl[j] : -__builtin_inf(); c.seq = live ? q[j] : 0ull; c.arg = i;
      const bool b1 = better(c, k1), b2 = better(c, k2);
      k2.sal = b1 ? k1.sal : (b2 ? c.sal : k2.sal); k2.seq = b1 ? k1.seq : (b2 ? c.seq : k2.seq); k2.arg = b1 ? k1.arg : (b2 ? c.arg : k2.arg);
      k1.sal = b1 ? c.sal : k1.sal; k1.seq = b1 ? c.seq : k1.seq; k1.arg = b1 ? c.arg : k1.arg;
    }
  };
  static_assert(kWinPer == 3, "batch_scan: one pass instance per number of blocks");
  const uint32_t nu = (uint32_t)__builtin_amdgcn_readfirstlane((int)n);
  if (nu > 2u * kGreedyThreads) pass(std::integral_constant<int, 3>{});
  else if (nu > kGreedyThreads) pass(std::integral_constant<int, 2>{});
  else pass(std::integral_constant<int, 1>{});
  SCAN_T(1);
  const int lane = tid & 63;
  const unsigned long long o1 = f64_ord(k1.sal), o2 = f64_ord(k2.sal);
  unsigned long long M1 = o1, M2 = o2;
  wave_top2_ord(M1, M2);
  const unsigned long long t1 = __ballot(o1 == M1), t1l = __ballot((o1 == M1) & (k1.seq != 0ull));
  const int l1 = (int)__builtin_ctzll(t1);
  const bool win1 = lane == l1;
  Key kk; kk.sal = win1 ? k2.sal : k1.sal; kk.seq = win1 ? k2.seq : k1.seq; kk.arg = win1 ? k2.arg : k1.arg;
  const unsigned long long oc = win1 ? o2 : o1;
  const unsigned long long t2 = __ballot(oc == M2), t2l = __ballot((oc == M2) & (kk.seq != 0ull));
  Key m1, m2;
  if (__popcll(t1) == 1 || t1l == 0ull) {
    m1 = lane_key(k1, l1);
    int src = (int)__builtin_ctzll(t2);
    if (__popcll(t2) != 1 && t2l != 0ull) {
#ifdef GLIA_HMT_PROFILE
      if (tid == 0) g_scanprof[5] += 1;
#endif
      const unsigned long long ms = wave_max_u64(oc == M2 ? kk.seq : 0ull);
      src = (int)__builtin_ctzll(__ballot((oc == M2) & (kk.seq == ms)));
    }
    m2 = lane_key(kk, src);
    SCAN_T(2);
  } else {
#ifdef GLIA_HMT_PROFILE
    if (tid == 0) g_scanprof[6] += 1;
#endif
    unsigned long long S1 = o1 == M1 ? k1.seq : 0ull, S2 = o2 == M1 ? k2.seq : 0ull;
    wave_top2_ord(S1, S2);
    const int w1 = (int)__builtin_ctzll(__ballot((o1 == M1) & (k1.seq == S1)));
    const bool winr = lane == w1;
    Key kc; kc.sal = winr ? k2.sal : k1.sal; kc.seq = winr ? k2.seq : k1.seq; kc.arg = winr ? k2.arg : k1.arg;
    const unsigned long long occ = winr ? o2 : o1;
    m1 = lane_key(k1, w1);
    m2 = lane_key(kc, (int)__builtin_ctzll(__ballot((occ == M1) & (kc.seq == S2))));
    SCAN_T(3);
  }
  if ((tid & 63) == 0) { b.part1[tid >> 6] = m1; b.part2[tid >> 6] = m2; }
  full_barrier();
  SCAN_T(4);
  if (tid == 0) { b.nkill = 0; b.kovf = 0; }
}

#ifdef GLIA_HMT_PROFILE
__device__ unsigned long long g_wideprof[8];
__device__ unsigned long long g_edgeprof[3][2];
#define WIDE_T(i) do { if (tid == 0) { const unsigned long long tn_ = __builtin_readcyclecounter(); g_wideprof[i] += tn_ - wt_; wt_ = tn_; } } while (0)
#else
#define WIDE_T(i) do {} while (0)
#endif
__device__ __forceinline__ uint32_t batch_contract_wide(const WinState& st, WinShared& w, WinWork& s, BatchShared& b, int tid, uint32_t slot, double rootsal,
                                                      unsigned long long k, unsigned long long ne, unsigned long long pool_used, double smin, double scale, uint32_t* newcount_out) {
  const uint32_t e = w.e[slot], r0 = w.u[slot], r1 = w.v[slot];
  const uint2 h0r = w.hu[slot], h1r = w.hv[slot];
  const uint32_t wn_now = w.n;
  const uint32_t off0 = h0r.x, len0 = h0r.y, off1 = h1r.x, len1 = h1r.y;
  const uint32_t total = len0 + len1;
  const uint32_t r2 = st.R0 + (uint32_t)k;
  const uint32_t r2off = (uint32_t)pool_used;
#ifdef GLIA_HMT_PROFILE
  unsigned long long wt_ = __builtin_readcyclecounter();
#endif
  lds_barrier();
  WIDE_T(0);
  if (tid == 0) {
    w.seq[slot] = 0;
    st.order[3 * k + 0] = r0; st.order[3 * k + 1] = r1; st.order[3 * k + 2] = r2;
    st.sal_out[k] = rootsal;
    st.er[e].seq = 0;
    st.rdead[r0] = 1; st.rdead[r1] = 1;
  }
  const bool small = total <= kMarkMax;
  win_stage_lists(st, s, tid, e, off0, len0, off1, len1, small);
  if (small) lds_barrier(); else full_barrier();
  WIDE_T(1);
  if (wn_now + total > st.wcap && wn_now > st.wcap / 2u) win_compact(w, tid, st.wcap);
  WIDE_T(2);
  const WinTau tau = {w.cthr, w.tsal, w.tseq, smin, scale};
  const uint32_t nwork = small ? s.nitems : total;
  const uint32_t lenR2 = small ? nwork : 0u;
  bool bad = false;
  uint32_t pend_e = kNone, pend_old = kNone;
#ifdef GLIA_HMT_PROFILE
  uint32_t ep_above = 0, ep_below = 0;
#endif
  auto rounds = [&](auto small_tag) {
    constexpr bool SMALL = decltype(small_tag)::value;
    for (uint32_t base = 0; base < nwork; base += kGreedyThreads) {
      const uint32_t i = base + tid;
      if (i >= nwork) break;
      FatEntry f0, f1;
      bool h0, h1;
      uint32_t rs;
      if (!win_match<SMALL>(st, s, i, e, off0, len0, off1, &rs, &h0, &h1, &f0, &f1)) continue;
      const uint32_t idx = atomicAdd(&s.newcount, 1u);
      const uint32_t newE = (uint32_t)ne + idx;
      double first;
      int second;
      if (mean_link(h0, f0.mean, (int)f0.n, h1, f1.mean, (int)f1.n, &first, &second)) bad = true;
      const uint32_t offRs = f0.off, posRs = f0.pos, lenRs = f0.len;
      if (h0 && h1) st.fpool[offRs + f1.pos].eid = kNone;
      const unsigned long long seq = update_seq(k, rs, r0, h0);
      const double sal = -first;
      const uint32_t cell = win_cell(sal, tau.smin, tau.scale, st.wB);
#ifdef GLIA_HMT_PROFILE
      if (cell < st.wch) ++ep_below; else ++ep_above;
#endif
      store_new_edge<true>(st, newE, rs, r2, posRs, idx, first, second, sal, seq, offRs, lenRs, r2off, lenR2, cell);
      win_queue_edge<true>(st, w, tau, newE, sal, seq, rs, r2, make_uint2(offRs, lenRs), make_uint2(r2off, lenR2), cell, pend_e, pend_old);
      if (h0) win_retire_edge<true, false, kBatchKill>(st, tau, f0.eid, -f0.mean, &b.nkill, b.kill, &b.kovf);
      if (h1) win_retire_edge<true, false, kBatchKill>(st, tau, f1.eid, -f1.mean, &b.nkill, b.kill, &b.kovf);
    }
  };
  if (small) rounds(std::true_type{}); else rounds(std::false_type{});
  if (bad) b.bad = 1;
  WIDE_T(3);
  if (small) lds_barrier(); else full_barrier();
  WIDE_T(4);
  const uint32_t newcount = s.newcount;
  if (!small) win_complete_r2<true>(st, tid, (uint32_t)ne, r2off, newcount, smin, scale);
  if (!small) for (uint32_t i = tid; i < (w.n < st.wcap ? w.n : st.wcap); i += kGreedyThreads) if (w.v[i] == r2) w.hv[i].y = newcount;
  if (pend_e != kNone) st.er[pend_e].next = pend_old;
  if (tid == 0) { st.adj_off[r2] = r2off; st.adj_len[r2] = newcount; }
  lds_barrier();
  WIDE_T(5);
#ifdef GLIA_HMT_PROFILE
  if (ep_above) atomicAdd(&g_edgeprof[small ? 1 : 2][0], (unsigned long long)ep_above);
  if (ep_below) atomicAdd(&g_edgeprof[small ? 1 : 2][1], (unsigned long long)ep_below);
#endif
  if (tid == 0) { s.nitems = 0; s.newcount = 0; }
  *newcount_out = newcount;
  return total;
}

__global__ __launch_bounds__(kGreedyThreads) void greedy_batch_kernel(WinState st) {
  __shared__ WinShared w;
  __shared__ WinWork s;
  __shared__ BatchShared b;
  const int tid = threadIdx.x, lane = tid & 63, wave = tid >> 6;
  unsigned long long k = st.ctrl[CTRL_MERGES], ne = st.ctrl[CTRL_EDGES], pool_used = st.ctrl[CTRL_ENTRIES];
  uint32_t status = ST_RUN;
  win_enter(st, w, s, tid);
  if (tid == 0) { b.nkill = 0; b.kovf = 0; b.bad = 0; }
  b.bitmap[wave][lane] = 0;
  if (tid < kNW) { Key z; z.sal = -__builtin_inf(); z.seq = 0; z.arg = 0; b.part1[tid] = z; b.part2[tid] = z; }
  full_barrier();
  const double smin = st.wrange[0], scale = st.wrange[1];
  uint32_t pend_e = kNone, pend_old = kNone;
  constexpr uint32_t kTab = kMarkSlots / kNW;
  uint32_t* const tk = &s.mk[wave * kTab]; uint32_t* const t0 = &s.mv0[wave * kTab]; uint32_t* const t1 = &s.mv1[wave * kTab];
  static_assert(sizeof(s.stage) >= (size_t)kNW * kTab * 20, "per-wave staging");
  uint32_t* const sg_eid = reinterpret_cast<uint32_t*>(&s.stage[0]) + wave * kTab;
  uint32_t* const sg_n = reinterpret_cast<uint32_t*>(&s.stage[0]) + (kNW + wave) * kTab;
  uint32_t* const sg_pos = reinterpret_cast<uint32_t*>(&s.stage[0]) + (2 * kNW + wave) * kTab;
  double* const sg_mean = reinterpret_cast<double*>(reinterpret_cast<uint32_t*>(&s.stage[0]) + 3 * kNW * kTab) + wave * kTab;
#ifdef GLIA_HMT_PROFILE
  unsigned long long bph[8] = {0, 0, 0, 0, 0, 0, 0, 0}, blast = __builtin_readcyclecounter(), brounds = 0, bmembers = 0, bvalid = 0, bwide = 0, bcut_sal = 0, bcut_dep = 0;
  unsigned long long bw_n[4] = {0, 0, 0, 0}, bw_cyc[4] = {0, 0, 0, 0}, bw_ent[4] = {0, 0, 0, 0}, bw_new[4] = {0, 0, 0, 0};
  uint32_t bep_above = 0, bep_below = 0;
  unsigned long long bsel[2] = {0, 0}, bsel_n[2] = {0, 0};
#define BPH0(wide) do { if (tid == 0) { unsigned long long tn = __builtin_readcyclecounter(); bph[0] += tn - blast; bsel[wide] += tn - blast; bsel_n[wide] += 1; blast = tn; } } while (0)
#define BPH(i) do { if (tid == 0) { unsigned long long tn = __builtin_readcyclecounter(); bph[i] += tn - blast; blast = tn; } } while (0)
#else
#define BPH(i) do {} while (0)
#define BPH0(wide) do {} while (0)
#endif

  for (unsigned long long it = 0; it < st.max_iters; ++it) {
    if (ne - st.ne_base > st.rebase_after) { status = ST_REBASE; break; }
    const int gi = lane >> 3, gj = lane & 7;
    const Key A = b.part1[gi], B = b.part1[gj], C = b.part2[gi];
    const unsigned long long beats = __ballot(better(A, B)), under = __ballot(better(C, B));
    const unsigned long long col = 0x0101010101010101ull << gj;
    const uint32_t rank = (uint32_t)__popcll(beats & col);
    const bool cand_ok = B.seq != 0 && (under & col) == 0;
    if (gi == 0 && cand_ok) b.byrank[rank] = (uint32_t)gj;
    const unsigned long long okmask = __ballot(gi == 0 && cand_ok);
    const uint32_t M = (uint32_t)__popcll(okmask);
    if (M == 0) {
      BPH(5);
      if (pend_e != kNone) { st.er[pend_e].next = pend_old; pend_e = kNone; }
      if (st.force_tree && k >= st.force_tree) { status = ST_NEED_TREE; break; }
      const int r = win_reload(st, w, tid, reinterpret_cast<double*>(&s.stage[0]), reinterpret_cast<unsigned long long*>(&s.stage[0]) + kSelMax);
      BPH(6);
      if (r == 1) { status = ST_DONE; break; }
      if (r == 2) { status = ST_NEED_TREE; break; }
      if (r == 3) { status = ST_REBASE; break; }
      batch_scan(st, w, b, tid, kScanOther);
      continue;
    }
    const unsigned long long minemask = __ballot(gi == 0 && cand_ok && rank == (uint32_t)wave);
    const bool member = minemask != 0;
    const int cj = member ? (int)__builtin_ctzll(minemask) : 0;
    const Key me = b.part1[cj];
    const uint32_t slot = me.arg;
    const uint32_t e = w.e[slot], r0 = w.u[slot], r1 = w.v[slot];
    const uint2 h0r = w.hu[slot], h1r = w.hv[slot];
    const uint32_t off0 = h0r.x, len0 = h0r.y, off1 = h1r.x, len1 = h1r.y;
    const uint32_t total = len0 + len1;
    if (k >= (unsigned long long)st.R0) { status = ST_INTERNAL; break; }
    const unsigned long long firstmask = __ballot(gi == 0 && cand_ok && rank == 0u);
    const Key top = b.part1[__builtin_ctzll(firstmask)];
    const uint2 th0 = w.hu[top.arg], th1 = w.hv[top.arg];
    const uint32_t top_total = th0.y + th1.y;
    BPH0(top_total > kMemMax ? 1 : 0);
    if (top_total > kMemMax) {
      if (ne + top_total > st.Ecap) { status = ST_NEED_EDGES; break; }
      if (pool_used + top_total > st.pool_cap) { status = ST_NEED_POOL; break; }
      uint32_t newcount = 0;
#ifdef GLIA_HMT_PROFILE
      const unsigned long long tw0 = __builtin_readcyclecounter();
#endif
      const uint32_t tt = batch_contract_wide(st, w, s, b, tid, top.arg, top.sal, k, ne, pool_used, smin, scale, &newcount);
      if (b.bad) { status = ST_BAD_SALIENCY; break; }
      k += 1; ne += newcount; pool_used += tt;
#ifdef GLIA_HMT_PROFILE
      bwide += 1;
      { const int cls = tt <= 512u ? 0 : tt <= kMarkMax ? 1 : tt <= 8192u ? 2 : 3; bw_n[cls] += 1; bw_cyc[cls] += __builtin_readcyclecounter() - tw0; bw_ent[cls] += tt; bw_new[cls] += newcount; }
#endif
      batch_scan(st, w, b, tid, kScanWide);
      if (w.spill_ord) { if (pend_e != kNone) { st.er[pend_e].next = pend_old; pend_e = kNone; } win_evict(st, w, tid); batch_scan(st, w, b, tid, kScanOther); }
      BPH(4);
      continue;
    }
    const bool narrow = member && total <= kMemMax;
    b.bitmap[wave][lane] = 0;
    FatEntry fe[kMemP];
    bool act[kMemP], side1[kMemP];
    uint32_t h[kMemP];
#pragma unroll
    for (int p = 0; p < kMemP; ++p) {
      const uint32_t i = (uint32_t)lane + 64u * (uint32_t)p;
      const bool inlist = narrow && i < total;
      side1[p] = i >= len0;
      fe[p].eid = kNone; fe[p].rs = 0; fe[p].n = 0; fe[p].pos = 0; fe[p].off = 0; fe[p].len = 0; fe[p].mean = 0.0;
      if (inlist) fe[p] = st.fpool[side1[p] ? off1 + (i - len0) : off0 + i];
      act[p] = inlist;
    }
    if (pend_e != kNone) { st.er[pend_e].next = pend_old; pend_e = kNone; }
#pragma unroll
    for (int p = 0; p < kMemP; ++p) {
      act[p] = act[p] && fe[p].eid != e && fe[p].eid != kNone;
      h[p] = (fe[p].rs * 2654435761u) >> 24;
      if (act[p]) {
        while (true) {
          const uint32_t old = atomicCAS(&tk[h[p]], 0u, fe[p].rs + 1u);
          if (old == 0u || old == fe[p].rs + 1u) break;
          h[p] = (h[p] + 1u) & (kTab - 1u);
        }
        if (side1[p]) {
          t1[h[p]] = 1u;
          sg_eid[h[p]] = fe[p].eid; sg_n[h[p]] = fe[p].n; sg_pos[h[p]] = fe[p].pos; sg_mean[h[p]] = fe[p].mean;
        } else t0[h[p]] = 1u;
        atomicOr(&b.bitmap[wave][(fe[p].rs >> 5) & 63u], 1u << (fe[p].rs & 31u));
      }
    }
    if (narrow && lane == 0) { atomicOr(&b.bitmap[wave][(r0 >> 5) & 63u], 1u << (r0 & 31u)); atomicOr(&b.bitmap[wave][(r1 >> 5) & 63u], 1u << (r1 & 31u)); }
    asm volatile("s_waitcnt lgkmcnt(0)" ::: "memory");
    bool owner[kMemP], both[kMemP];
    uint32_t p_eid[kMemP], p_n[kMemP], p_pos[kMemP];
    double p_mean[kMemP];
#pragma unroll
    for (int p = 0; p < kMemP; ++p) {
      const uint32_t m0 = act[p] ? t0[h[p]] : 0u, m1 = act[p] ? t1[h[p]] : 0u;
      owner[p] = act[p] && (!side1[p] || m0 == 0u);
      both[p] = owner[p] && !side1[p] && m1 != 0u;
      p_eid[p] = sg_eid[h[p]]; p_n[p] = sg_n[h[p]]; p_pos[p] = sg_pos[h[p]]; p_mean[p] = sg_mean[h[p]];
    }
#pragma unroll
    for (int p = 0; p < kMemP; ++p) if (act[p]) { tk[h[p]] = 0u; t0[h[p]] = 0u; t1[h[p]] = 0u; }
    double first[kMemP]; int second[kMemP]; uint32_t idx[kMemP];
    bool bad = false;
    uint32_t newcount = 0;
    double mx = -__builtin_inf();
#pragma unroll
    for (int p = 0; p < kMemP; ++p) {
      const bool h0 = owner[p] && !side1[p], h1 = owner[p] && (side1[p] || both[p]);
      bad = mean_link(h0, fe[p].mean, (int)fe[p].n, h1, both[p] ? p_mean[p] : fe[p].mean, both[p] ? (int)p_n[p] : (int)fe[p].n, &first[p], &second[p]) || bad;
      const double f = first[p];
      const unsigned long long ownmask = __ballot(owner[p]);
      idx[p] = newcount + (uint32_t)__popcll(ownmask & ((1ull << lane) - 1ull));
      newcount += (uint32_t)__popcll(ownmask);
      mx = (owner[p] && -f > mx) ? -f : mx;
    }
#pragma unroll
    for (int d = 32; d >= 1; d >>= 1) { const double o = __shfl_xor(mx, d); mx = o > mx ? o : mx; }
    if (lane == 0) { b.m_newcount[wave] = narrow ? newcount : 0u; b.m_total[wave] = narrow ? total : 0xFFFFFFFFu; b.m_maxsal[wave] = mx; }
    if (bad) b.bad = 1;
    const uint32_t wn_round = w.n;
    lds_barrier();
    BPH(1);
    if (b.bad) { status = ST_BAD_SALIENCY; break; }
    uint32_t V, ne_off, pool_off, my_ne, my_pool;
    {
      const uint32_t j = (uint32_t)lane & 7u;
      const Key kj = b.part1[b.byrank[j]];
      const uint32_t u = w.u[kj.arg], v = w.v[kj.arg];
      const uint32_t tj = b.m_total[j], nj = b.m_newcount[j];
      double pm = -__builtin_inf();
      uint32_t hit = 0, pre_n = 0, pre_t = 0;
#pragma unroll
      for (uint32_t i = 0; i < (uint32_t)kNW; ++i) {
        const double ms = b.m_maxsal[i];
        const uint32_t bu = b.bitmap[i][(u >> 5) & 63u], bv = b.bitmap[i][(v >> 5) & 63u];
        const uint32_t ti = b.m_total[i], ni = b.m_newcount[i];
        if (i < j) { pm = ms > pm ? ms : pm; hit |= ((bu >> (u & 31u)) | (bv >> (v & 31u))) & 1u; pre_n += ni; pre_t += ti; }
      }
      const bool okj = j < M && tj != 0xFFFFFFFFu && (j == 0u || (kj.sal > pm && hit == 0u));
      const uint32_t okbits = (uint32_t)(__ballot(lane < kNW && okj) & 0xFFull);
      V = (uint32_t)__builtin_ctz(~okbits);
#ifdef GLIA_HMT_PROFILE
      if (V < M) { const uint32_t cutsal = (uint32_t)(__ballot(lane < kNW && j == V && !(kj.sal > pm)) & 0xFFull); if (cutsal) bcut_sal += 1; else bcut_dep += 1; }
#endif
      my_ne = (uint32_t)__builtin_amdgcn_readlane((int)pre_n, wave); my_pool = (uint32_t)__builtin_amdgcn_readlane((int)pre_t, wave);
      const uint32_t last = V - 1u;
      ne_off = (uint32_t)__shfl((int)(pre_n + nj), (int)last); pool_off = (uint32_t)__shfl((int)(pre_t + tj), (int)last);
    }
    const uint32_t sum_tot = pool_off;
    if (ne + sum_tot > st.Ecap) { status = ST_NEED_EDGES; break; }
    if (pool_used + sum_tot > st.pool_cap) { status = ST_NEED_POOL; break; }
    bool popped = false;
    if (wn_round + ne_off > st.wcap && wn_round > st.wcap / 2u) {
      if ((uint32_t)wave < V && lane == 0) w.seq[slot] = 0;
      popped = true;
      lds_barrier();
      win_compact(w, tid, st.wcap);
    }
    const WinTau tau = {w.cthr, w.tsal, w.tseq, smin, scale};
    BPH(2);
    if ((uint32_t)wave < V) {
      const unsigned long long kk = k + (unsigned long long)wave;
      const uint32_t r2 = st.R0 + (uint32_t)kk;
      const uint32_t r2off = (uint32_t)pool_used + my_pool;
      if (lane == 0) {
        if (!popped) w.seq[slot] = 0;
        st.order[3 * kk + 0] = r0; st.order[3 * kk + 1] = r1; st.order[3 * kk + 2] = r2;
        st.sal_out[kk] = me.sal;
        st.er[e].seq = 0;
        st.rdead[r0] = 1; st.rdead[r1] = 1;
        st.adj_off[r2] = r2off; st.adj_len[r2] = newcount;
      }
#pragma unroll
      for (int p = 0; p < kMemP; ++p) {
        if (!owner[p]) continue;
        const bool h0 = !side1[p];
        const uint32_t rs = fe[p].rs;
        const uint32_t newE = (uint32_t)ne + my_ne + idx[p];
        const uint32_t offRs = fe[p].off, posRs = fe[p].pos, lenRs = fe[p].len;
        if (both[p]) st.fpool[offRs + p_pos[p]].eid = kNone;
        const unsigned long long seq = update_seq(kk, rs, r0, h0);
        const double sal = -first[p];
        const uint32_t cell = win_cell(sal, tau.smin, tau.scale, st.wB);
#ifdef GLIA_HMT_PROFILE
        if (cell < st.wch) ++bep_below; else ++bep_above;
#endif
        store_new_edge<true>(st, newE, rs, r2, posRs, idx[p], first[p], second[p], sal, seq, offRs, lenRs, r2off, newcount, cell);
        win_queue_edge<true>(st, w, tau, newE, sal, seq, rs, r2, make_uint2(offRs, lenRs), make_uint2(r2off, newcount), cell, pend_e, pend_old);
        win_retire_edge<true, false, kBatchKill>(st, tau, fe[p].eid, -fe[p].mean, &b.nkill, b.kill, &b.kovf);
        if (both[p]) win_retire_edge<true, false, kBatchKill>(st, tau, p_eid[p], -p_mean[p], &b.nkill, b.kill, &b.kovf);
      }
    }
    lds_barrier();
    BPH(3);
#ifdef GLIA_HMT_PROFILE
    brounds += 1; bmembers += M; bvalid += V;
#endif
    k += V; ne += ne_off; pool_used += pool_off;
    batch_scan(st, w, b, tid, kScanNarrow);
    if (w.spill_ord) { if (pend_e != kNone) { st.er[pend_e].next = pend_old; pend_e = kNone; } win_evict(st, w, tid); batch_scan(st, w, b, tid, kScanOther); }
    BPH(4);
  }
#ifdef GLIA_HMT_PROFILE
  if (bep_above) atomicAdd(&g_edgeprof[0][0], (unsigned long long)bep_above);
  if (bep_below) atomicAdd(&g_edgeprof[0][1], (unsigned long long)bep_below);
  full_barrier();
  if (tid == 0) printf("[batch profile] created edges at or above / below the horizon (cumulative): narrow commit %llu / %llu  wide on the LDS table %llu / %llu  wide on the global marks %llu / %llu\n",
                       atomicAdd(&g_edgeprof[0][0], 0ull), atomicAdd(&g_edgeprof[0][1], 0ull), atomicAdd(&g_edgeprof[1][0], 0ull), atomicAdd(&g_edgeprof[1][1], 0ull),
                       atomicAdd(&g_edgeprof[2][0], 0ull), atomicAdd(&g_edgeprof[2][1], 0ull));
  if (tid == 0) printf("[batch profile] merges %llu: select %llu  compute %llu  validate %llu  commit %llu  scan %llu  loop-top %llu  reload %llu (cycles); rounds %llu candidates %llu committed %llu (cut by saliency %llu, by adjacency %llu) wide %llu\n",
                       k, bph[0], bph[1], bph[2], bph[3], bph[4], bph[5], bph[6], brounds, bmembers, bvalid, bcut_sal, bcut_dep, bwide);
  if (tid == 0) printf("[batch profile] scan phases (cumulative cycles, wave 0): loads %llu  compare %llu  top2 %llu  top2 with a tied best %llu  barrier %llu  calls %llu  tied second %llu  tied best %llu\n",
                       g_scanprof[0], g_scanprof[1], g_scanprof[2], g_scanprof[3], g_scanprof[4], g_scanprof[7], g_scanprof[5], g_scanprof[6]);
  if (tid == 0) printf("[batch profile] scan fill (cumulative; n <= 512, <= 1024, more): after reload/evict %llu %llu %llu  after narrow round %llu %llu %llu  after wide %llu %llu %llu\n",
                       g_scanfill[0][0], g_scanfill[0][1], g_scanfill[0][2], g_scanfill[1][0], g_scanfill[1][1], g_scanfill[1][2], g_scanfill[2][0], g_scanfill[2][1], g_scanfill[2][2]);
  if (tid == 0) printf("[batch profile] loop top (this launch): narrow rounds %llu cycles %llu  wide pops %llu cycles %llu\n", bsel_n[0], bsel[0], bsel_n[1], bsel[1]);
  if (tid == 0) printf("[batch profile] wide phases (cumulative cycles): entry-barrier %llu  lists+table %llu  compact %llu  main loop (wave 0) %llu  loop barrier %llu  tail %llu\n",
                       g_wideprof[0], g_wideprof[1], g_wideprof[2], g_wideprof[3], g_wideprof[4], g_wideprof[5]);
  if (tid == 0) printf("[batch profile] wide by entries (<=512, <=1408, <=8192, more): n %llu %llu %llu %llu  cycles %llu %llu %llu %llu  entries %llu %llu %llu %llu  new edges %llu %llu %llu %llu\n",
                       bw_n[0], bw_n[1], bw_n[2], bw_n[3], bw_cyc[0], bw_cyc[1], bw_cyc[2], bw_cyc[3], bw_ent[0], bw_ent[1], bw_ent[2], bw_ent[3], bw_new[0], bw_new[1], bw_new[2], bw_new[3]);
#endif
  if (pend_e != kNone) st.er[pend_e].next = pend_old;
  full_barrier();
  win_leave(st, w, tid, k, ne, pool_used, status);
}

}
}
```

### glia_amd/csrc/greedy_window.hpp

```cpp
#pragma once
#include "greedy_tree.hpp"
#include "edge_record.hpp"

namespace glia {
namespace {

static_assert(kRecNone == kNone, "edge_record.hpp");
struct WinState {
  EdgeRec* er; FatEntry* fpool;
  uint32_t* whead;
  uint32_t* wcnt;
  const uint32_t* isort; const unsigned long long* isort_seq;
  const uint32_t* ige;
  const double* wrange;
  uint32_t* order; double* sal_out; unsigned long long* ctrl;
  unsigned long long* rsz; double* rsum; uint32_t *mark0, *mark1, *adj_off, *adj_len;
  unsigned long long pool_cap, max_iters, cond_t0, cond_t1;
  double cond_rpb;
  uint32_t R0, Ecap, wB, nsort;
  unsigned long long ne_base, rebase_after;
  uint32_t wcap, wbudget;
  int cond_n;
  uint32_t wch;
  uint8_t* rdead;
  unsigned long long force_tree;
  uint8_t* ecat;
};
constexpr uint32_t kWinCap = 1536;
constexpr uint32_t kWinBudget = 768;
constexpr uint32_t kWinMinLoad = 192;
constexpr uint32_t kWinMinPartial = 96;
constexpr uint32_t kKillMax = 8;
constexpr int kNW = kGreedyThreads / 64;
constexpr int kWinPer = (int)(kWinCap / kGreedyThreads);
static_assert(kWinPer * kGreedyThreads == (int)kWinCap, "window capacity");
struct WinShared {
  double sal[kWinCap];
  unsigned long long seq[kWinCap];
  uint32_t e[kWinCap], u[kWinCap], v[kWinCap];
  uint2 hu[kWinCap], hv[kWinCap];
  int cthr; uint32_t iptr;
  double tsal; unsigned long long tseq;
  alignas(16) uint32_t n;
  uint32_t nk, kovf, pad0;
  alignas(16) uint32_t kill[kKillMax];
  alignas(16) Key part[kNW];
  uint32_t touched[2][64];
  uint32_t wsum[kNW];
  uint32_t bcast, maxcell, err, need_tree;
  double psal; unsigned long long pseq;
  unsigned long long spill_ord;
};
struct WinWork {
  uint32_t mk[kMarkSlots], mv0[kMarkSlots], mv1[kMarkSlots];
  uint32_t items[kMarkMax], newidx[kMarkMax], nitems, newcount, bad;
  FatEntry stage[kMarkMax];
};

__host__ __device__ __forceinline__ uint32_t win_cell(double sal, double smin, double scale, uint32_t B) {
  double t = (sal - smin) * scale;
  t = t > 0.0 ? t : 0.0;
  return t >= (double)(B - 1u) ? B - 1u : (uint32_t)t;
}
__device__ __forceinline__ bool win_above(int cthr, double tsal, unsigned long long tseq, int cell, double sal, unsigned long long seq) {
  return cell > cthr || (cell == cthr && (sal > tsal || (sal == tsal && seq > tseq)));
}

__device__ __forceinline__ uint32_t block_scan_incl(uint32_t v, uint32_t* wsum, int tid, uint32_t* total) {
  const int lane = tid & 63, wave = tid >> 6;
  uint32_t x = v;
#pragma unroll
  for (int d = 1; d < 64; d <<= 1) { const uint32_t y = (uint32_t)__shfl_up((int)x, d); if (lane >= d) x += y; }
  full_barrier();
  if (lane == 63) wsum[wave] = x;
  full_barrier();
  uint32_t base = 0, tot = 0;
#pragma unroll
  for (int i = 0; i < kNW; ++i) { const uint32_t s = wsum[i]; if (i < wave) base += s; tot += s; }
  *total = tot;
  return base + x;
}

__device__ __forceinline__ void win_put(WinShared& w, uint32_t slot, double sal, unsigned long long seq, uint32_t e, uint32_t u, uint32_t v, uint2 hu, uint2 hv) {
  w.sal[slot] = sal; w.seq[slot] = seq; w.e[slot] = e; w.u[slot] = u; w.v[slot] = v; w.hu[slot] = hu; w.hv[slot] = hv;
}
__device__ __forceinline__ void win_take(const WinState& st, WinShared& w, uint32_t e, const EdgeRec& r) {
  if (r.seq != 0) {
    const uint32_t slot = atomicAdd(&w.n, 1u);
    if (slot < st.wcap) win_put(w, slot, r.sal, r.seq, e, r.u, r.v, r.hu, r.hv); else w.err = 1;
  }
}

__device__ __forceinline__ void win_scan(const WinState& st, WinShared& w, int tid, uint32_t r2, uint32_t r2len) {
  const uint4 hd = *reinterpret_cast<const uint4*>(&w.n);
  const uint4 k0 = *reinterpret_cast<const uint4*>(&w.kill[0]), k1 = *reinterpret_cast<const uint4*>(&w.kill[4]);
  unsigned long long q[kWinPer]; uint32_t e[kWinPer], v[kWinPer]; double sl[kWinPer];
#pragma unroll
  for (int j = 0; j < kWinPer; ++j) { const uint32_t i = (uint32_t)tid + (uint32_t)j * kGreedyThreads; q[j] = w.seq[i]; e[j] = w.e[i]; v[j] = w.v[i]; sl[j] = w.sal[i]; }
  const uint32_t n = hd.x, nk = hd.y < kKillMax ? hd.y : kKillMax;
  const uint32_t kl[kKillMax] = {k0.x, k0.y, k0.z, k0.w, k1.x, k1.y, k1.z, k1.w};
  Key k;
  k.sal = -__builtin_inf(); k.seq = 0; k.arg = 0;
#pragma unroll
  for (int j = 0; j < kWinPer; ++j) {
    const uint32_t i = (uint32_t)tid + (uint32_t)j * kGreedyThreads;
    bool live = i < n && q[j] != 0;
    bool dead = false;
    if (nk) {
#pragma unroll
      for (uint32_t t = 0; t < kKillMax; ++t) dead = dead || (t < nk && kl[t] == e[j]);
    }
    if (live && hd.z) dead = dead || st.er[e[j]].seq == 0;
    if (live && dead) { w.seq[i] = 0; live = false; }
    if (live && v[j] == r2) w.hv[i].y = r2len;
    Key c; c.sal = live ? sl[j] : -__builtin_inf(); c.seq = live ? q[j] : 0ull; c.arg = i;
    if (better(c, k)) k = c;
  }
  k = wave_max(k);
  if ((tid & 63) == 0) w.part[tid >> 6] = k;
  lds_barrier();
  if (tid == 0) { w.nk = 0; w.kovf = 0; }
}
__device__ __forceinline__ Key win_root(const WinShared& w, int lane) {
  static_assert(kNW == 8, "win_root");
  Key k = w.part[lane & (kNW - 1)];
  key_max_step<0xB1>(k); key_max_step<0x4E>(k);
  const Key a = lane_key(k, 0), b = lane_key(k, 4);
  return better(b, a) ? b : a;
}

__device__ __forceinline__ uint32_t win_compact(WinShared& w, int tid, uint32_t cap = kWinCap) {
  double sal[kWinPer]; unsigned long long seq[kWinPer]; uint32_t e[kWinPer], u[kWinPer], v[kWinPer]; uint2 hu[kWinPer], hv[kWinPer];
  uint32_t live = 0;
  const uint32_t n = w.n < cap ? w.n : cap;
#pragma unroll
  for (int j = 0; j < kWinPer; ++j) {
    const uint32_t i = (uint32_t)tid * kWinPer + j;
    seq[j] = i < n ? w.seq[i] : 0ull;
    sal[j] = w.sal[i]; e[j] = w.e[i]; u[j] = w.u[i]; v[j] = w.v[i]; hu[j] = w.hu[i]; hv[j] = w.hv[i];
    live += seq[j] != 0;
  }
  uint32_t total;
  uint32_t o = block_scan_incl(live, w.wsum, tid, &total) - live;
#pragma unroll
  for (int j = 0; j < kWinPer; ++j) if (seq[j] != 0) { win_put(w, o, sal[j], seq[j], e[j], u[j], v[j], hu[j], hv[j]); ++o; }
  if (tid == 0) w.n = total;
  full_barrier();
  return total;
}

__device__ __forceinline__ void win_push_global(const WinState& st, uint32_t e, uint32_t cell) {
  const uint32_t old = atomicExch(&st.whead[cell], e);
  st.er[e].next = old;
  atomicAdd(&st.wcnt[cell], 1u);
}

__device__ __forceinline__ void win_flush(const WinState& st, WinShared& w, int tid) {
  const double smin = st.wrange[0], scale = st.wrange[1];
  if (tid == 0) w.maxcell = 0;
  full_barrier();
  const uint32_t n = w.n < st.wcap ? w.n : st.wcap;
  uint32_t mc = 0;
  for (uint32_t i = tid; i < n; i += kGreedyThreads) {
    if (w.seq[i] == 0) continue;
    const uint32_t c = win_cell(w.sal[i], smin, scale, st.wB);
    win_push_global(st, w.e[i], c);
    mc = mc > c + 1u ? mc : c + 1u;
  }
  if (mc) atomicMax(&w.maxcell, mc);
  full_barrier();
  if (tid == 0) {
    if (w.maxcell && (int)w.maxcell - 1 >= w.cthr) { w.cthr = (int)w.maxcell - 1; w.tsal = __builtin_inf(); w.tseq = ~0ull; }
    w.n = 0;
  }
  full_barrier();
}

__device__ __forceinline__ void win_evict(const WinState& st, WinShared& w, int tid) {
  const double smin = st.wrange[0], scale = st.wrange[1];
  const double lim = f64_unord(w.spill_ord);
  const uint32_t n = w.n < st.wcap ? w.n : st.wcap;
  full_barrier();
  for (uint32_t i = tid; i < n; i += kGreedyThreads) {
    if (w.seq[i] == 0 || w.sal[i] > lim) continue;
    win_push_global(st, w.e[i], win_cell(w.sal[i], smin, scale, st.wB));
    w.seq[i] = 0;
  }
  full_barrier();
  if (tid == 0) { w.n = n; w.cthr = (int)win_cell(lim, smin, scale, st.wB); w.tsal = lim; w.tseq = ~0ull; w.spill_ord = 0; }
  full_barrier();
}

__device__ __forceinline__ void win_take_initial(const WinState& st, WinShared& w, uint32_t a, uint32_t b, int tid) {
  for (uint32_t i = a + (uint32_t)tid; i < b; i += kGreedyThreads) { const uint32_t e = st.isort[i]; const EdgeRec r = st.er[e]; win_take(st, w, e, r); }
}

constexpr uint32_t kSelMax = 384;
__device__ __forceinline__ int win_reload(const WinState& st, WinShared& w, int tid, double* sel_sal, unsigned long long* sel_seq) {
  full_barrier();
  if (tid == 0) { w.n = 0; w.need_tree = 0; }
  full_barrier();
  uint32_t c_hi = (uint32_t)(w.cthr + 1) < st.wB ? (uint32_t)(w.cthr + 1) : st.wB, loaded = 0, iptr = w.iptr;
  int result = 1;
  const uint32_t c_floor = st.wch < st.wB ? st.wch : 0u;
  while (c_hi > c_floor) {
    const bool valid = (uint32_t)tid < c_hi - c_floor;
    const uint32_t c = valid ? c_hi - 1u - (uint32_t)tid : 0u;
    const uint32_t cn = valid ? ld_relaxed(&st.wcnt[c]) : 0u;
    uint32_t total;
    const uint32_t incl = block_scan_incl(cn, w.wsum, tid, &total);
    const bool ok = valid && incl <= st.wbudget - loaded;
    const uint32_t m = (uint32_t)__syncthreads_count(ok ? 1 : 0);
    const uint32_t nvalid = c_hi - c_floor < (uint32_t)kGreedyThreads ? c_hi - c_floor : (uint32_t)kGreedyThreads;
    if (m != 0) {
      const uint32_t c_lo = c_hi - m;
      if ((uint32_t)tid == m - 1u) w.bcast = incl;
      const uint32_t i_to = st.ige[c_lo];
      win_take_initial(st, w, iptr, i_to, tid);
      iptr = i_to > iptr ? i_to : iptr;
      if ((uint32_t)tid < m) {
        uint32_t e = ld_relaxed(&st.whead[c]);
        if (e != kNone) {
          st_agent(&st.whead[c], kNone);
          if (cn != 0) while (e != kNone) { const EdgeRec r = st.er[e]; win_take(st, w, e, r); e = r.next; }
        }
        if (cn != 0) st_agent(&st.wcnt[c], 0u);
      }
      full_barrier();
      loaded += w.bcast;
      c_hi = c_lo;
      if (loaded) result = 0;
    }
    if (m < nvalid) {
      const uint32_t room = st.wbudget - loaded;
      const uint32_t cs = c_hi - 1u;
      if (room >= (kWinMinPartial < st.wbudget / 8u ? kWinMinPartial : st.wbudget / 8u) || loaded == 0) {
        const uint32_t K = (room / 2u < kSelMax ? room / 2u : kSelMax) > 1u ? (room / 2u < kSelMax ? room / 2u : kSelMax) : 2u, RA = room > K ? room - K : 1u;
        const uint32_t seg_end = st.ige[cs];
        const uint32_t before = w.n;
        if (tid == 0) {
          uint32_t hn = 0, nlive = 0;
          for (uint32_t e = ld_relaxed(&st.whead[cs]); e != kNone;) {
            const EdgeRec r = st.er[e];
            if (r.seq != 0) {
              ++nlive;
              if (hn < K) {
                uint32_t i = hn++;
                while (i > 0) {
                  const uint32_t p = (i - 1u) >> 1;
                  if (!(sel_sal[p] > r.sal || (sel_sal[p] == r.sal && sel_seq[p] > r.seq))) break;
                  sel_sal[i] = sel_sal[p]; sel_seq[i] = sel_seq[p]; i = p;
                }
                sel_sal[i] = r.sal; sel_seq[i] = r.seq;
              } else if (r.sal > sel_sal[0] || (r.sal == sel_sal[0] && r.seq > sel_seq[0])) {
                uint32_t i = 0;
                while (true) {
                  uint32_t c = 2u * i + 1u;
                  if (c >= hn) break;
                  if (c + 1u < hn && (sel_sal[c + 1u] < sel_sal[c] || (sel_sal[c + 1u] == sel_sal[c] && sel_seq[c + 1u] < sel_seq[c]))) ++c;
                  if (!(sel_sal[c] < r.sal || (sel_sal[c] == r.sal && sel_seq[c] < r.seq))) break;
                  sel_sal[i] = sel_sal[c]; sel_seq[i] = sel_seq[c]; i = c;
                }
                sel_sal[i] = r.sal; sel_seq[i] = r.seq;
              }
            }
            e = r.next;
          }
          w.psal = nlive > K ? sel_sal[0] : -__builtin_inf(); w.pseq = nlive > K ? sel_seq[0] : 0ull;
        }
        full_barrier();
        double tsal = w.psal; unsigned long long tseq = w.pseq;
        const uint32_t iA = seg_end > iptr ? (seg_end - iptr < RA ? seg_end : iptr + RA) : iptr;
        if (iA < seg_end) {
          const uint32_t et = st.isort[iA]; const double as = st.er[et].sal; const unsigned long long aq = st.isort_seq[iA];
          if (as > tsal || (as == tsal && aq > tseq)) { tsal = as; tseq = aq; }
        }
        if (tid == 0) w.bcast = 0;
        full_barrier();
        uint32_t mine = 0;
        for (uint32_t i = iptr + (uint32_t)tid; i < iA; i += kGreedyThreads) {
          const uint32_t e = st.isort[i]; const EdgeRec r = st.er[e];
          const unsigned long long q = st.isort_seq[i];
          if (r.sal > tsal || (r.sal == tsal && q > tseq)) { ++mine; win_take(st, w, e, r); }
        }
        if (mine) atomicAdd(&w.bcast, mine);
        full_barrier();
        iptr += w.bcast;
        if (tid == 0) {
          uint32_t keep_head = kNone, keep_tail = kNone;
          for (uint32_t e = ld_relaxed(&st.whead[cs]); e != kNone;) {
            const EdgeRec r = st.er[e];
            if (r.seq != 0) {
              if (r.sal > tsal || (r.sal == tsal && r.seq > tseq)) win_take(st, w, e, r);
              else { if (keep_head == kNone) keep_head = e; else st.er[keep_tail].next = e; keep_tail = e; }
            }
            e = r.next;
          }
          if (keep_tail != kNone) st.er[keep_tail].next = kNone;
          st_agent(&st.whead[cs], keep_head);
        }
        full_barrier();
        const uint32_t moved = w.n - before;
        if (moved == 0u && w.bcast == 0u) {
          full_barrier();
          if (tid == 0) st_agent(&st.wcnt[cs], 0u);
          c_hi = cs;
          continue;
        }
        if (tid == 0) { if (moved) atomicSub(&st.wcnt[cs], moved); w.cthr = (int)cs; w.tsal = tsal; w.tseq = tseq; w.iptr = iptr; }
        if (moved || w.bcast) result = 0;
        full_barrier();
        return result;
      }
      break;
    }
    if (loaded >= (kWinMinLoad < st.wbudget / 4u ? kWinMinLoad : st.wbudget / 4u)) break;
  }
  full_barrier();
  if (tid == 0 && result != 2) { w.cthr = (int)c_hi - 1; w.tsal = __builtin_inf(); w.tseq = ~0ull; w.iptr = iptr; }
  full_barrier();
  if (result == 1 && c_floor != 0u) result = 3;
  return result;
}

struct WinTau { int cthr; double tsal; unsigned long long tseq; double smin, scale; };

__device__ __forceinline__ void win_stage_lists(const WinState& st, WinWork& s, int tid, uint32_t e, uint32_t off0, uint32_t len0, uint32_t off1, uint32_t len1, bool small) {
  const uint32_t total = len0 + len1;
  for (uint32_t i = tid; i < total; i += kGreedyThreads) {
    const bool side1 = i >= len0;
    const FatEntry fe = st.fpool[side1 ? off1 + (i - len0) : off0 + i];
    if (fe.eid == e || fe.eid == kNone) continue;
    if (small) {
      s.stage[i] = fe;
      uint32_t h = (fe.rs * 2654435761u) >> 21;
      while (true) {
        const uint32_t old = atomicCAS(&s.mk[h], 0u, fe.rs + 1u);
        if (old == 0u) { s.items[atomicAdd(&s.nitems, 1u)] = h; break; }
        if (old == fe.rs + 1u) break;
        h = (h + 1u) & (kMarkSlots - 1u);
      }
      (side1 ? s.mv1 : s.mv0)[h] = i + 1u;
    } else (side1 ? st.mark1 : st.mark0)[fe.rs] = i + 1u;
  }
}
template <bool SMALL>
__device__ __forceinline__ bool win_match(const WinState& st, WinWork& s, uint32_t i, uint32_t e, uint32_t off0, uint32_t len0, uint32_t off1,
                                          uint32_t* rs, bool* h0, bool* h1, FatEntry* f0, FatEntry* f1) {
  if constexpr (SMALL) {
    const uint32_t h = s.items[i];
    *rs = s.mk[h] - 1u;
    const uint32_t m0 = s.mv0[h], m1 = s.mv1[h];
    s.mk[h] = 0u; s.mv0[h] = 0u; s.mv1[h] = 0u;
    *h0 = m0 != 0; *h1 = m1 != 0;
    *f0 = s.stage[*h0 ? m0 - 1u : m1 - 1u]; *f1 = s.stage[*h1 ? m1 - 1u : m0 - 1u];
  } else {
    const bool side1 = i >= len0;
    const FatEntry fe = st.fpool[side1 ? off1 + (i - len0) : off0 + i];
    if (fe.eid == e || fe.eid == kNone) return false;
    *rs = fe.rs;
    if (!side1) {
      const uint32_t m = st.mark1[fe.rs];
      *h0 = true; *h1 = m != 0; *f0 = fe;
      *f1 = *h1 ? st.fpool[off1 + (m - 1u - len0)] : fe;
    } else {
      if (st.mark0[fe.rs] != 0u) return false;
      *h0 = false; *h1 = true; *f0 = fe; *f1 = fe;
    }
  }
  return true;
}
template <bool BATCH>
__device__ __forceinline__ void store_new_edge(const WinState& st, uint32_t newE, uint32_t rs, uint32_t r2, uint32_t posRs, uint32_t idx, double first, int second,
                                               double sal, unsigned long long seq, uint32_t offRs, uint32_t lenRs, uint32_t r2off, uint32_t lenR2, uint32_t cell) {
  if (BATCH && cell < st.wch) st.ecat[newE] = (uint8_t)((uint32_t)(seq >> 30) & 3u);
  else {
    uint4* pq4 = reinterpret_cast<uint4*>(&st.er[newE]);
    pq4[0] = make_uint4(rs, r2, posRs, idx);
    const unsigned long long mb = (unsigned long long)__double_as_longlong(first);
    pq4[1] = make_uint4((uint32_t)mb, (uint32_t)(mb >> 32), (uint32_t)second, kNone);
    pq4[2] = make_uint4(offRs, lenRs, r2off, lenR2);
    const unsigned long long sbits = (unsigned long long)__double_as_longlong(sal);
    pq4[3] = make_uint4((uint32_t)sbits, (uint32_t)(sbits >> 32), (uint32_t)seq, (uint32_t)(seq >> 32));
  }
  FatEntry a; a.eid = newE; a.rs = r2; a.n = (uint32_t)second; a.pos = idx; a.off = r2off; a.len = lenR2; a.mean = first;
  st.fpool[offRs + posRs] = a;
  FatEntry b; b.eid = newE; b.rs = rs; b.n = (uint32_t)second; b.pos = posRs; b.off = offRs; b.len = lenRs; b.mean = first;
  st.fpool[r2off + idx] = b;
}
template <bool BATCH>
__device__ __forceinline__ void win_queue_edge(const WinState& st, WinShared& w, const WinTau& tau, uint32_t newE, double sal, unsigned long long seq, uint32_t rs, uint32_t r2,
                                               uint2 hrs, uint2 hr2, uint32_t cell, uint32_t& pend_e, uint32_t& pend_old) {
  const bool above = win_above(tau.cthr, tau.tsal, tau.tseq, (int)cell, sal, seq);
  uint32_t sl = kWinCap;
  if (above) {
    sl = atomicAdd(&w.n, 1u);
    if (!BATCH || sl < st.wcap) win_put(w, sl, sal, seq, newE, rs, r2, hrs, hr2);
    else atomicMax(&w.spill_ord, f64_ord(sal));
  }
  if (BATCH ? (sl >= st.wcap && (above || cell >= st.wch)) : !above) {
    if (pend_e != kNone) st.er[pend_e].next = pend_old;
    pend_e = newE; pend_old = atomicExch(&st.whead[cell], newE);
    atomicAdd(&st.wcnt[cell], 1u);
  }
}
template <bool BATCH, bool COND, uint32_t KMAX>
__device__ __forceinline__ void win_retire_edge(const WinState& st, const WinTau& tau, uint32_t de, double dsal, uint32_t* nkill, uint32_t* kill, uint32_t* kovf) {
  const uint32_t dc = win_cell(dsal, tau.smin, tau.scale, st.wB);
  const bool tie = (int)dc == tau.cthr && dsal == tau.tsal;
  unsigned long long dq = BATCH ? 0ull : 1ull;
  if (BATCH && dc < st.wch) return;
  if (!BATCH && (COND || tie)) dq = st.er[de].seq;
  st.er[de].seq = 0;
  if (!BATCH && dq == 0) return;
  if ((BATCH && tie) || win_above(tau.cthr, tau.tsal, tau.tseq, (int)dc, dsal, dq)) {
    const uint32_t j = atomicAdd(nkill, 1u); if (j < KMAX) kill[j] = de; else *kovf = 1;
  } else atomicSub(&st.wcnt[dc], 1u);
}
template <bool BATCH>
__device__ __forceinline__ void win_complete_r2(const WinState& st, int tid, uint32_t ne, uint32_t r2off, uint32_t newcount, double smin, double scale) {
  for (uint32_t j = tid; j < newcount; j += kGreedyThreads) {
    const FatEntry fb = st.fpool[r2off + j];
    st.fpool[fb.off + fb.pos].len = newcount;
    if (!BATCH || win_cell(-fb.mean, smin, scale, st.wB) >= st.wch) st.er[ne + j].hv.y = newcount;
    st.mark0[fb.rs] = 0; st.mark1[fb.rs] = 0;
  }
}
__device__ __forceinline__ void win_enter(const WinState& st, WinShared& w, WinWork& s, int tid) {
  if (tid == 0) {
    w.n = 0; w.nk = 0; w.kovf = 0; w.err = 0; w.spill_ord = 0; s.nitems = 0; s.newcount = 0; s.bad = 0;
    w.cthr = (int)(long long)st.ctrl[CTRL_CTHR]; w.tsal = __longlong_as_double((long long)st.ctrl[CTRL_TSAL]); w.tseq = st.ctrl[CTRL_TSEQ]; w.iptr = (uint32_t)st.ctrl[CTRL_IPTR];
  }
  for (uint32_t i = tid; i < kMarkSlots; i += kGreedyThreads) { s.mk[i] = 0; s.mv0[i] = 0; s.mv1[i] = 0; }
  for (uint32_t i = tid; i < kWinCap; i += kGreedyThreads) { w.seq[i] = 0; w.e[i] = 0; w.v[i] = 0; w.sal[i] = 0.0; }
}
__device__ __forceinline__ void win_leave(const WinState& st, WinShared& w, int tid, unsigned long long k, unsigned long long ne, unsigned long long pool_used, uint32_t status) {
  win_flush(st, w, tid);
  if (tid == 0) {
    st.ctrl[CTRL_MERGES] = k; st.ctrl[CTRL_EDGES] = ne; st.ctrl[CTRL_ENTRIES] = pool_used;
    st.ctrl[CTRL_STATUS] = w.err ? (unsigned long long)ST_INTERNAL : status; st.ctrl[CTRL_WERR] = w.err; st.ctrl[CTRL_WFILL] = w.n;
    st.ctrl[CTRL_CTHR] = (unsigned long long)(long long)w.cthr; st.ctrl[CTRL_TSAL] = (unsigned long long)__double_as_longlong(w.tsal); st.ctrl[CTRL_TSEQ] = w.tseq; st.ctrl[CTRL_IPTR] = w.iptr;
  }
}

template <bool COND>
__global__ __launch_bounds__(kGreedyThreads) void greedy_window_kernel(WinState st) {
  __shared__ WinShared w;
  __shared__ WinWork s;
  const int tid = threadIdx.x, lane = tid & 63;
  unsigned long long k = st.ctrl[CTRL_MERGES], ne = st.ctrl[CTRL_EDGES], pool_used = st.ctrl[CTRL_ENTRIES];
  uint32_t status = ST_RUN;
  win_enter(st, w, s, tid);
  if (tid < 128) w.touched[tid >> 6][tid & 63] = 0;
  if (tid < kNW) { w.part[tid].sal = -__builtin_inf(); w.part[tid].seq = 0; w.part[tid].arg = 0; }
  full_barrier();
  const double smin = st.wrange[0], scale = st.wrange[1];
  uint32_t r2prev = kNone;
#ifdef GLIA_HMT_PROFILE
  unsigned long long wph[8] = {0, 0, 0, 0, 0, 0, 0, 0}, wlast = __builtin_readcyclecounter(), wtiter = wlast;
  unsigned long long wtb[5] = {0, 0, 0, 0, 0}, wnb[5] = {0, 0, 0, 0, 0}, wdb[5] = {0, 0, 0, 0, 0}, wreloads = 0, wcompacts = 0, wloaded = 0, winwin = 0, wdeps = 0;
#define WPH(i) do { if (tid == 0) { unsigned long long tn = __builtin_readcyclecounter(); wph[i] += tn - wlast; wlast = tn; } } while (0)
#else
#define WPH(i) do {} while (0)
#endif

  for (unsigned long long it = 0; it < st.max_iters; ++it) {
    const Key root = win_root(w, lane);
    if (root.seq == 0) {
      WPH(5);
      if (st.force_tree && k >= st.force_tree) { status = ST_NEED_TREE; break; }
      const int r = win_reload(st, w, tid, reinterpret_cast<double*>(&s.stage[0]), reinterpret_cast<unsigned long long*>(&s.stage[0]) + kSelMax);
#ifdef GLIA_HMT_PROFILE
      wreloads += 1; wloaded += w.n;
#endif
      WPH(6);
      if (r == 1) { status = ST_DONE; break; }
      if (r == 2) { status = ST_NEED_TREE; break; }
      if (r == 3) { status = ST_REBASE; break; }
      win_scan(st, w, tid, kNone, 0);
      r2prev = kNone;
      continue;
    }
    const uint32_t slot = root.arg;
    const uint32_t e = w.e[slot], r0 = w.u[slot], r1 = w.v[slot];
    const uint2 h0r = w.hu[slot], h1r = w.hv[slot];
    const uint32_t wn_now = w.n;
    const int cthr = w.cthr; const double tsal = w.tsal; const unsigned long long tseq = w.tseq;
    const uint32_t off0 = h0r.x, len0 = h0r.y, off1 = h1r.x, len1 = h1r.y;
    const uint32_t total = len0 + len1;
    if (k >= (unsigned long long)st.R0) { status = ST_INTERNAL; break; }
    const uint32_t r2 = st.R0 + (uint32_t)k;
    const uint32_t r2off = (uint32_t)pool_used;
    const int par = (int)(k & 1ull);
    const uint32_t tb0 = w.touched[par ^ 1][(r0 >> 5) & 63u], tb1 = w.touched[par ^ 1][(r1 >> 5) & 63u];
    const bool dep = r2prev != kNone && (r1 == r2prev || r0 == r2prev || ((tb0 >> (r0 & 31u)) & 1u) || ((tb1 >> (r1 & 31u)) & 1u));
    if (dep) {
      full_barrier();
#ifdef GLIA_HMT_PROFILE
      wdeps += 1;
#endif
    }
    WPH(0);
    if (COND) {
      unsigned long long sz0 = st.rsz[r0], sz1 = st.rsz[r1]; double su0 = st.rsum[r0], su1 = st.rsum[r1];
      const unsigned long long z2 = sz0 + sz1; const double w2 = su0 + su1;
      if (sz0 > sz1) { const unsigned long long t = sz0; sz0 = sz1; sz1 = t; const double d = su0; su0 = su1; su1 = d; }
      bool ok = sz0 < st.cond_t0;
      if (!ok && st.cond_n > 1) {
        if (sz0 < st.cond_t1 && sdivide(su0, (double)sz0, 0.0) > st.cond_rpb) ok = true;
        if (!ok && sz1 < st.cond_t1 && sdivide(su1, (double)sz1, 0.0) > st.cond_rpb) ok = true;
      }
      if (!ok) {
        full_barrier();
        if (tid == 0) { w.seq[slot] = 0; st.er[e].seq = 0; }
        full_barrier();
        win_scan(st, w, tid, kNone, 0);
        continue;
      }
      if (tid == 0) { st.rsz[r2] = z2; st.rsum[r2] = w2; }
    }
    if (ne + total > st.Ecap) { status = ST_NEED_EDGES; break; }
    if (pool_used + total > st.pool_cap) { status = ST_NEED_POOL; break; }
    if (tid == 0) {
      w.seq[slot] = 0;
      st.order[3 * k + 0] = r0; st.order[3 * k + 1] = r1; st.order[3 * k + 2] = r2;
      st.sal_out[k] = root.sal;
      st.er[e].seq = 0;
    }
    if (tid >= 64 && tid < 128) w.touched[par][tid & 63] = 0;
    const bool small = total <= kMarkMax;

    win_stage_lists(st, s, tid, e, off0, len0, off1, len1, small);
    full_barrier();
    WPH(1);
    if (wn_now + total > st.wcap) {
#ifdef GLIA_HMT_PROFILE
      wcompacts += 1;
#endif
      const uint32_t wn_live = win_compact(w, tid, st.wcap);
      if (wn_live + total > st.wcap) {
        win_flush(st, w, tid);
        if (total > st.wcap) {
          if (tid == 0) { w.cthr = (int)st.wB; w.tsal = __builtin_inf(); w.tseq = ~0ull; }
          full_barrier();
        }
      }
    }
    const bool moved = wn_now + total > st.wcap;
    const WinTau tau = {moved ? w.cthr : cthr, moved ? w.tsal : tsal, moved ? w.tseq : tseq, smin, scale};
    const uint32_t nwork = small ? s.nitems : total;
    WPH(2);

    bool bad = false;
    uint32_t pend_e = kNone, pend_old = kNone;
    for (uint32_t base = 0; base < nwork; base += kGreedyThreads) {
      const uint32_t i = base + tid;
      if (i >= nwork) break;
      FatEntry f0, f1;
      bool h0, h1;
      uint32_t rs;
      if (!(small ? win_match<true>(st, s, i, e, off0, len0, off1, &rs, &h0, &h1, &f0, &f1) : win_match<false>(st, s, i, e, off0, len0, off1, &rs, &h0, &h1, &f0, &f1))) continue;
      const uint32_t idx = atomicAdd(&s.newcount, 1u);
      const uint32_t newE = (uint32_t)ne + idx;
      atomicOr(&w.touched[par][(rs >> 5) & 63u], 1u << (rs & 31u));
      double first;
      int second;
      if (mean_link(h0, f0.mean, (int)f0.n, h1, f1.mean, (int)f1.n, &first, &second)) bad = true;
      const uint32_t offRs = f0.off, posRs = f0.pos, lenRs = f0.len;
      if (h0 && h1) st.fpool[offRs + f1.pos].eid = kNone;
      const unsigned long long seq = update_seq(k, rs, r0, h0);
      const double sal = -first;
      const uint32_t cell = win_cell(sal, tau.smin, tau.scale, st.wB);
      store_new_edge<false>(st, newE, rs, r2, posRs, idx, first, second, sal, seq, offRs, lenRs, r2off, 0u, cell);
      if (small) { s.items[i] = offRs + posRs; s.newidx[i] = idx; }
      win_queue_edge<false>(st, w, tau, newE, sal, seq, rs, r2, make_uint2(offRs, lenRs), make_uint2(r2off, 0u), cell, pend_e, pend_old);
      if (h0) win_retire_edge<false, COND, kKillMax>(st, tau, f0.eid, -f0.mean, &w.nk, w.kill, &w.kovf);
      if (h1) win_retire_edge<false, COND, kKillMax>(st, tau, f1.eid, -f1.mean, &w.nk, w.kill, &w.kovf);
    }
    if (bad) s.bad = 1;
    if (small) lds_barrier(); else full_barrier();
    if (s.bad) { if (pend_e != kNone) st.er[pend_e].next = pend_old; status = ST_BAD_SALIENCY; break; }
    WPH(3);
    const uint32_t newcount = s.newcount;
    if (small) {
      for (uint32_t i = tid; i < nwork; i += kGreedyThreads) { st.fpool[s.items[i]].len = newcount; st.er[(uint32_t)ne + s.newidx[i]].hv.y = newcount; }
    } else {
      win_complete_r2<false>(st, tid, (uint32_t)ne, r2off, newcount, smin, scale);
    }
    if (w.kovf) full_barrier(); else lds_barrier();
    if (tid == 0) { st.adj_off[r2] = r2off; st.adj_len[r2] = newcount; s.nitems = 0; s.newcount = 0; }
    win_scan(st, w, tid, r2, newcount);
    if (pend_e != kNone) st.er[pend_e].next = pend_old;
    r2prev = r2;
    WPH(4);
#ifdef GLIA_HMT_PROFILE
    if (tid == 0) {
      const unsigned long long tn = __builtin_readcyclecounter();
      const int b = total <= 64 ? 0 : total <= 512 ? 1 : total <= kMarkMax ? 2 : total <= 8192 ? 3 : 4;
      wtb[b] += tn - wtiter; wnb[b] += 1; wdb[b] += total; wtiter = tn; winwin += w.n;
    }
#endif
    k += 1; ne += newcount; pool_used += total;
  }
#ifdef GLIA_HMT_PROFILE
  if (tid == 0) printf("[window profile] merges %llu: pop %llu  lists+table %llu  room %llu  build %llu  finish+scan %llu  loop-top %llu  reload %llu (cycles); reloads %llu (items %llu) compactions %llu dependent %llu; mean window fill %llu\n",
                       k, wph[0], wph[1], wph[2], wph[3], wph[4], wph[5], wph[6], wreloads, wloaded, wcompacts, wdeps, k ? winwin / k : 0ull);
  if (tid == 0) printf("[window profile] by width (<=64, <=512, <=1408, <=8192, more): merges %llu %llu %llu %llu %llu  cycles %llu %llu %llu %llu %llu  entries %llu %llu %llu %llu %llu\n",
                       wnb[0], wnb[1], wnb[2], wnb[3], wnb[4], wtb[0], wtb[1], wtb[2], wtb[3], wtb[4], wdb[0], wdb[1], wdb[2], wdb[3], wdb[4]);
#endif
  full_barrier();
  win_leave(st, w, tid, k, ne, pool_used, status);
}

}
}
```

Baseline: 323,100.

## Pack edge category into list entry pos; derive seqs from lists, narrow collect lanes

Stores the 2-bit seq category in the top bits of each adjacency-list entry's pos field, removes the separate ecat array, and lets the list-based collection compute each edge's seq directly from the entry instead of reading the edge record. Adds a collect kernel variant that assigns 16 lanes per region when lists are short, plus an initial-collection kernel that fills seqs without scanning. The aim is to cut scattered global reads and idle lanes during rebaseline collection. It limits list positions to 30 bits and adds an optional check mode and profiling counters.

```diff
diff --git a/cli/edge_rebuild_check.cpp b/cli/edge_rebuild_check.cpp
--- a/cli/edge_rebuild_check.cpp
+++ b/cli/edge_rebuild_check.cpp
@@ -19,7 +19,7 @@
     const E& g = edges[e];
     const uint32_t pu = cur[g.u]++, pv = cur[g.v]++;
     FatEntry a; a.eid = (uint32_t)e; a.rs = g.v; a.n = g.n; a.pos = pv; a.off = off[g.v]; a.len = deg[g.v]; a.mean = g.mean;
-    FatEntry b = a; b.rs = g.u; b.pos = pu; b.off = off[g.u]; b.len = deg[g.u];
+    FatEntry b = a; b.rs = g.u; b.pos = pack_pos(pu, g.u < g.r0 ? 0u : (g.h0 ? 1u : 2u)); b.off = off[g.u]; b.len = deg[g.u];
     pool[off[g.u] + pu] = a; pool[off[g.v] + pv] = b;
     posu[e] = pu; posv[e] = pv;
   }
@@ -37,7 +37,7 @@
       memcpy(&mb, &first, 8); memcpy(&sb, &sal, 8);
       const uint32_t want[16] = {rs, r2, posu[fe.eid], posv[fe.eid], (uint32_t)mb, (uint32_t)(mb >> 32), g.n, kRecNone,
                                  off[rs], deg[rs], off[r2], deg[r2], (uint32_t)sb, (uint32_t)(sb >> 32), (uint32_t)seq, (uint32_t)(seq >> 32)};
-      const EdgeRec got = rebuild_edge_record(fe, i, v, off[v], deg[v], (uint32_t)((seq >> 30) & 3u), R0);
+      const EdgeRec got = rebuild_edge_record(fe, i, v, off[v], deg[v], R0);
       if (memcmp(&got, want, 64) != 0) {
         const uint32_t* w = reinterpret_cast<const uint32_t*>(&got);
         printf("edge_rebuild_check: edge %u (%u, %u) differs:", fe.eid, rs, r2);
diff --git a/cli/entry_seq_check.cpp b/cli/entry_seq_check.cpp
--- /dev/null
+++ b/cli/entry_seq_check.cpp
@@ -0,0 +1,69 @@
+#include <cstdio>
+#include <cstring>
+#include "../glia_amd/csrc/edge_record.hpp"
+
+using namespace glia;
+
+static int fail(const char* what, unsigned long long a, unsigned long long b) {
+  printf("entry_seq_check: %s: %llx / %llx\n", what, a, b);
+  return 1;
+}
+
+int main() {
+  int packed = 0;
+  const uint32_t positions[3] = {0u, 1u, (1u << 30) - 1u};
+  for (uint32_t pos : positions)
+    for (uint32_t cat = 0; cat < 4; ++cat) {
+      FatEntry fe;
+      memset(&fe, 0, sizeof(fe));
+      fe.pos = pack_pos(pos, cat);
+      if (entry_pos(fe) != pos) return fail("position after pack_pos", entry_pos(fe), pos);
+      if (entry_cat(fe) != cat) return fail("cat bits after pack_pos", entry_cat(fe), cat);
+      if (fe.pos != (pos | (cat << 30))) return fail("layout of the packed field", fe.pos, pos | (cat << 30));
+      ++packed;
+    }
+
+  const uint32_t R0 = 1000, E0 = 3000;
+  struct C { uint32_t rs, k, cat, posRs, idx, n; double mean; uint32_t offRs, lenRs, r2off, lenR2, eid; };
+  const C cs[] = {{17, 0, 0, 5, 0, 7, 0.125, 40, 9, 9000, 3, 3000},
+                  {999, 41, 1, 0, 2, 3, 0.5, 7700, 1, 9100, 4, 3100},
+                  {1003, 41, 2, 8191, 3, 11, 0.33203125, 123456, 8200, 9100, 4, 3101},
+                  {12, 998, 1, (1u << 30) - 1u, 0, 1, 0.99609375, 16, 1u << 30, 50000, 1, 70000},
+                  {1500, 900, 0, 1, 1, 40, 0.0, 300, 2, 60000, 2, 65000}};
+  int rebuilt = 0, cats[3] = {0, 0, 0}, top = 0;
+  for (const C& c : cs) {
+    const uint32_t r2 = R0 + c.k;
+    const unsigned long long seq = ((unsigned long long)(c.k + 1u) << 32) | ((unsigned long long)c.cat << 30) | c.rs;
+    const double first = c.mean, sal = -first;
+    unsigned long long mb, sb;
+    memcpy(&mb, &first, 8); memcpy(&sb, &sal, 8);
+    const uint32_t want[16] = {c.rs, r2, c.posRs, c.idx, (uint32_t)mb, (uint32_t)(mb >> 32), c.n, kRecNone,
+                               c.offRs, c.lenRs, c.r2off, c.lenR2, (uint32_t)sb, (uint32_t)(sb >> 32), (uint32_t)seq, (uint32_t)(seq >> 32)};
+    FatEntry b; b.eid = c.eid; b.rs = c.rs; b.n = c.n; b.pos = pack_pos(c.posRs, c.cat); b.off = c.offRs; b.len = c.lenRs; b.mean = first;
+    const EdgeRec got = rebuild_edge_record(b, c.idx, r2, c.r2off, c.lenR2, R0);
+    if (memcmp(&got, want, 64) != 0) {
+      const uint32_t* w = reinterpret_cast<const uint32_t*>(&got);
+      printf("entry_seq_check: created edge (%u, %u) differs:", c.rs, r2);
+      for (int j = 0; j < 16; ++j) printf(" %08x/%08x", w[j], want[j]);
+      printf("\n");
+      return 1;
+    }
+    if (entry_seq(b, r2, E0, R0) != seq) return fail("entry_seq of a created edge", entry_seq(b, r2, E0, R0), seq);
+    ++rebuilt; ++cats[c.cat]; top += c.posRs == (1u << 30) - 1u;
+  }
+  if (!cats[0] || !cats[1] || !cats[2] || top != 1) return fail("cases", (unsigned long long)rebuilt, (unsigned long long)top);
+
+  int initial = 0;
+  const uint32_t slots[3] = {0u, 1u, E0 - 1u};
+  for (uint32_t e : slots)
+    for (uint32_t cat = 0; cat < 4; ++cat) {
+      FatEntry fe;
+      memset(&fe, 0, sizeof(fe));
+      fe.eid = e; fe.rs = 3; fe.pos = pack_pos(77, cat);
+      if (entry_seq(fe, 5, E0, R0) != (unsigned long long)e + 1ull) return fail("entry_seq of an initial edge", entry_seq(fe, 5, E0, R0), e + 1ull);
+      ++initial;
+    }
+  printf("entry_seq_check: %d packed fields round-trip, %d records rebuilt from packed entries agree with the stored form (cat 0/1/2: %d/%d/%d, at position 2^30-1: %d), %d initial seqs\n",
+         packed, rebuilt, cats[0], cats[1], cats[2], top, initial);
+  return 0;
+}
diff --git a/glia_amd/csrc/api.cpp b/glia_amd/csrc/api.cpp
--- a/glia_amd/csrc/api.cpp
+++ b/glia_amd/csrc/api.cpp
@@ -17,7 +17,8 @@
 
 static const char* const kOptionKeys[] = {"GLIA_HMT_PB_WINDOW", "GLIA_HMT_PB_BATCH", "GLIA_HMT_WINCAP", "GLIA_HMT_REBASE", "GLIA_HMT_HORIZON",
                                           "GLIA_HMT_FORCE_TREE", "GLIA_HMT_HELPERS", "GLIA_HMT_TRACE", "GLIA_HMT_LIBM", "GLIA_HMT_BC_NOCOMMON",
-                                          "GLIA_HMT_BC_GENERIC", "GLIA_HMT_DEBUG", "GLIA_HMT_MAXITERS", "GLIA_HMT_MINCAP", "GLIA_HMT_MEDIAN_BATCH", "GLIA_HMT_BCFEAT", "GLIA_HMT_CC"};
+                                          "GLIA_HMT_BC_GENERIC", "GLIA_HMT_DEBUG", "GLIA_HMT_MAXITERS", "GLIA_HMT_MINCAP", "GLIA_HMT_MEDIAN_BATCH", "GLIA_HMT_BCFEAT", "GLIA_HMT_CC",
+                                          "GLIA_HMT_COLLECT_LANES", "GLIA_HMT_COLLECT_CHECK"};
 static std::mutex g_opt_mu;
 static std::unordered_map<std::string, std::string> g_opt;
 static bool g_opt_init = false;
diff --git a/glia_amd/csrc/edge_record.hpp b/glia_amd/csrc/edge_record.hpp
--- a/glia_amd/csrc/edge_record.hpp
+++ b/glia_amd/csrc/edge_record.hpp
@@ -35,13 +35,24 @@
 };
 static_assert(sizeof(EdgeRec) == 64, "EdgeRec layout");
 
-GLIA_REC_HD inline EdgeRec rebuild_edge_record(const FatEntry& fe, uint32_t idx, uint32_t v, uint32_t voff, uint32_t vlen, uint32_t cat, uint32_t R0) {
+constexpr uint32_t kPosBits = 30;
+constexpr uint32_t kPosMask = (1u << kPosBits) - 1u;
+GLIA_REC_HD inline uint32_t pack_pos(uint32_t pos, uint32_t cat) { return (pos & kPosMask) | (cat << kPosBits); }
+GLIA_REC_HD inline uint32_t entry_pos(const FatEntry& fe) { return fe.pos & kPosMask; }
+GLIA_REC_HD inline uint32_t entry_cat(const FatEntry& fe) { return fe.pos >> kPosBits; }
+
+GLIA_REC_HD inline unsigned long long entry_seq(const FatEntry& fe, uint32_t v, uint32_t E0, uint32_t R0) {
+  if (fe.eid < E0) return (unsigned long long)fe.eid + 1ull;
+  return ((unsigned long long)(v - R0 + 1u) << 32) | ((unsigned long long)entry_cat(fe) << kPosBits) | fe.rs;
+}
+
+GLIA_REC_HD inline EdgeRec rebuild_edge_record(const FatEntry& fe, uint32_t idx, uint32_t v, uint32_t voff, uint32_t vlen, uint32_t R0) {
   EdgeRec r;
-  r.u = fe.rs; r.v = v; r.posu = fe.pos; r.posv = idx;
+  r.u = fe.rs; r.v = v; r.posu = entry_pos(fe); r.posv = idx;
   r.mean = fe.mean; r.n = (int)fe.n; r.next = kRecNone;
   r.hu.x = fe.off; r.hu.y = fe.len; r.hv.x = voff; r.hv.y = vlen;
   r.sal = -fe.mean;
-  r.seq = ((unsigned long long)(v - R0 + 1u) << 32) | ((unsigned long long)(cat & 3u) << 30) | fe.rs;
+  r.seq = ((unsigned long long)(v - R0 + 1u) << 32) | ((unsigned long long)entry_cat(fe) << kPosBits) | fe.rs;
   return r;
 }
 
diff --git a/glia_amd/csrc/greedy.hip b/glia_amd/csrc/greedy.hip
--- a/glia_amd/csrc/greedy.hip
+++ b/glia_amd/csrc/greedy.hip
@@ -70,25 +70,36 @@
   const uint32_t i = atomicAdd(counter, 1u);
   kseq[i] = q; vals[i] = e;
 }
-__global__ void win_collect_lists_kernel(WinState st, uint32_t n_regions, unsigned long long* kseq, uint32_t* vals, uint32_t cap, uint32_t* counter) {
-  const uint32_t r = (blockIdx.x * blockDim.x + threadIdx.x) >> 6, lane = threadIdx.x & 63u;
-  if (r >= n_regions || st.rdead[r]) return;
-  const uint32_t off = st.adj_off[r], len = st.adj_len[r];
+__global__ void win_collect_initial_kernel(uint32_t E0, unsigned long long* kseq, uint32_t* vals) {
+  const uint32_t i = blockIdx.x * blockDim.x + threadIdx.x;
+  if (i < E0) { kseq[i] = (unsigned long long)i + 1ull; vals[i] = i; }
+}
+template <int LANES, bool CHECK>
+__global__ void win_collect_lists_kernel(WinState st, uint32_t n_regions, uint32_t E0, unsigned long long* kseq, uint32_t* vals, uint32_t cap, uint32_t* counter) {
+  static_assert(LANES == 16 || LANES == 64, "lanes per region");
+  constexpr uint32_t kGroups = 64u / (uint32_t)LANES;
+  const uint32_t wv = (blockIdx.x * blockDim.x + threadIdx.x) >> 6, lane = threadIdx.x & 63u;
+  const uint32_t r = wv * kGroups + lane / (uint32_t)LANES, sub = lane % (uint32_t)LANES;
+  const bool alive = r < n_regions && !st.rdead[r];
+  const uint32_t off = alive ? st.adj_off[r] : 0u, len = alive ? st.adj_len[r] : 0u;
+  uint32_t maxlen = len;
+#pragma unroll
+  for (int d = LANES; d < 64; d <<= 1) { const uint32_t o = (uint32_t)__shfl_xor((int)maxlen, d); maxlen = o > maxlen ? o : maxlen; }
   const double smin = st.wrange[0], scale = st.wrange[1];
-  uint32_t rebuilt = 0;
-  for (uint32_t base = 0; base < len; base += 64u) {
-    const uint32_t i = base + lane;
+  uint32_t rebuilt = 0, compared = 0, wrong = 0;
+  for (uint32_t base = 0; base < maxlen; base += (uint32_t)LANES) {
+    const uint32_t i = base + sub;
     unsigned long long q = 0;
     uint32_t e = kNone;
     if (i < len) {
       const FatEntry fe = st.fpool[off + i];
       if (fe.eid != kNone && fe.rs < r && !st.rdead[fe.rs]) {
         e = fe.eid;
+        q = entry_seq(fe, r, E0, st.R0);
         if ((unsigned long long)e >= st.ne_base && win_cell(-fe.mean, smin, scale, st.wB) < st.wch) {
-          const EdgeRec rec = rebuild_edge_record(fe, i, r, off, len, st.ecat[e], st.R0);
-          st.er[e] = rec;
-          q = rec.seq; ++rebuilt;
-        } else q = st.er[e].seq;
+          st.er[e] = rebuild_edge_record(fe, i, r, off, len, st.R0);
+          ++rebuilt;
+        } else if (CHECK) { ++compared; wrong += st.er[e].seq != q; }
       }
     }
     const unsigned long long m = __ballot(q != 0);
@@ -101,6 +112,8 @@
     if (q != 0 && o < cap) { kseq[o] = q; vals[o] = e; }
   }
   if (rebuilt) atomicAdd(&counter[1], rebuilt);
+  if (CHECK && compared) atomicAdd(&counter[2], compared);
+  if (CHECK && wrong) atomicAdd(&counter[3], wrong);
 }
 __global__ void win_salkey_kernel(const EdgeRec* er, const uint32_t* vals, uint32_t n, unsigned long long* ksal) {
   const uint32_t i = blockIdx.x * blockDim.x + threadIdx.x;
@@ -129,8 +142,8 @@
   const uint32_t u = g.e_u[e], v = g.e_v[e];
   const uint32_t pu = atomicAdd(&cursor[u], 1u), pv = atomicAdd(&cursor[v], 1u);
   const uint32_t ou = g.adj_off[u], ov = g.adj_off[v], lu = g.adj_len[u], lv = g.adj_len[v];
-  FatEntry a; a.eid = e; a.rs = v; a.n = (uint32_t)g.e_n[e]; a.pos = pv; a.off = ov; a.len = lv; a.mean = g.e_mean[e];
-  FatEntry b = a; b.rs = u; b.pos = pu; b.off = ou; b.len = lu;
+  FatEntry a; a.eid = e; a.rs = v; a.n = (uint32_t)g.e_n[e]; a.pos = pack_pos(pv, 0u); a.off = ov; a.len = lv; a.mean = g.e_mean[e];
+  FatEntry b = a; b.rs = u; b.pos = pack_pos(pu, 0u); b.off = ou; b.len = lu;
   st.fpool[ou + pu] = a; g.e_posu[e] = pu;
   st.fpool[ov + pv] = b; g.e_posv[e] = pv;
   EdgeRec r; r.u = u; r.v = v; r.posu = pu; r.posv = pv; r.mean = g.e_mean[e]; r.n = g.e_n[e]; r.next = kNone;
@@ -277,6 +290,10 @@
   double horizon_factor = 0.0;
   bool from_lists = false;
   unsigned long long rebuilt_last = 0;
+  uint32_t prev_n = 0;
+  int force_lanes = 0;
+  const char* horizon_rule = "none";
+  bool check = false, trace = false;
 
   int init(DeviceBuffers& buf, WinState& ws, const double* leaf_sal, uint32_t n_initial, uint32_t B, uint32_t R, hipStream_t stream) {
     int rc;
@@ -296,7 +313,7 @@
     if ((rc = buf.get(&ksal2, E0, false, stream))) return rc;
     if ((rc = buf.get(&vals, E0, false, stream))) return rc;
     if ((rc = buf.get(&vals2, E0, false, stream))) return rc;
-    if ((rc = buf.get(&counter, 2, true, stream))) return rc;
+    if ((rc = buf.get(&counter, 4, true, stream))) return rc;
     GLIA_HIP_TRY(rocprim::radix_sort_pairs_desc(nullptr, tmp_bytes, kseq, kseq2, vals, vals2, (size_t)E0, 0, 64, stream));
     if ((rc = buf.get((char**)&tmp, tmp_bytes ? tmp_bytes : 16, false, stream))) return rc;
     ws.wrange = range; ws.isort = isort; ws.isort_seq = iseq; ws.ige = ige;
@@ -310,20 +327,36 @@
     return GLIA_HMT_OK;
   }
   int collect(const WinState& ws, uint32_t n_edges, uint32_t n_regions, hipStream_t stream, uint32_t* n_out) {
-    GLIA_HIP_TRY(hipMemsetAsync(counter, 0, 2 * sizeof(uint32_t), stream));
-    if (from_lists) hipLaunchKernelGGL(win_collect_lists_kernel, dim3((unsigned)(((unsigned long long)n_regions * 64ull + 255ull) / 256ull)), dim3(256), 0, stream, ws, n_regions, kseq, vals, E0, counter);
-    else hipLaunchKernelGGL(win_collect_kernel, dim3((n_edges + 255) / 256), dim3(256), 0, stream, ws.er, n_edges, ws.rdead, kseq, vals, counter);
+    GLIA_HIP_TRY(hipMemsetAsync(counter, 0, 4 * sizeof(uint32_t), stream));
+    if (from_lists) {
+      const unsigned long long live_regions = 2ull * ws.R0 > n_regions ? 2ull * ws.R0 - n_regions : 1ull;
+      const int lanes = force_lanes ? force_lanes : 2ull * prev_n <= 16ull * live_regions ? 16 : 64;
+      const dim3 grid((unsigned)(((unsigned long long)n_regions * (unsigned long long)lanes + 255ull) / 256ull)), block(256);
+      if (check) {
+        if (lanes == 16) hipLaunchKernelGGL((win_collect_lists_kernel<16, true>), grid, block, 0, stream, ws, n_regions, E0, kseq, vals, E0, counter);
+        else hipLaunchKernelGGL((win_collect_lists_kernel<64, true>), grid, block, 0, stream, ws, n_regions, E0, kseq, vals, E0, counter);
+      } else if (lanes == 16) hipLaunchKernelGGL((win_collect_lists_kernel<16, false>), grid, block, 0, stream, ws, n_regions, E0, kseq, vals, E0, counter);
+      else hipLaunchKernelGGL((win_collect_lists_kernel<64, false>), grid, block, 0, stream, ws, n_regions, E0, kseq, vals, E0, counter);
+    } else hipLaunchKernelGGL(win_collect_kernel, dim3((n_edges + 255) / 256), dim3(256), 0, stream, ws.er, n_edges, ws.rdead, kseq, vals, counter);
     GLIA_HIP_TRY(hipGetLastError());
-    uint32_t h[2] = {0, 0};
+    uint32_t h[4] = {0, 0, 0, 0};
     GLIA_HIP_TRY(hipMemcpyAsync(h, counter, sizeof(h), hipMemcpyDeviceToHost, stream));
     GLIA_HIP_TRY(hipStreamSynchronize(stream));
     if (h[0] > E0) { set_error("greedy: more live edges than initial edges (internal error)"); return GLIA_HMT_ERR_INTERNAL; }
+    if (check && from_lists) {
+      if (trace) fprintf(stderr, "[trace] collection check: %u seqs compared with their records, %u disagree\n", h[2], h[3]);
+      if (h[3]) { set_error("greedy: " + std::to_string(h[3]) + " list entries give another seq than their edge records (internal error)"); return GLIA_HMT_ERR_INTERNAL; }
+    }
     *n_out = h[0]; rebuilt_last = h[1];
     return GLIA_HMT_OK;
   }
-  int rebaseline(WinState& ws, uint32_t n_edges, unsigned long long* ctrl, hipStream_t stream) {
+  int rebaseline(WinState& ws, uint32_t n_edges, unsigned long long* ctrl, hipStream_t stream, bool initial = false) {
     uint32_t n = 0;
-    if (int rc = collect(ws, n_edges, ws.R0 + (uint32_t)ctrl[CTRL_MERGES], stream, &n)) return rc;
+    if (initial) {
+      n = E0;
+      hipLaunchKernelGGL(win_collect_initial_kernel, dim3((E0 + 255) / 256), dim3(256), 0, stream, E0, kseq, vals);
+    } else if (int rc = collect(ws, n_edges, ws.R0 + (uint32_t)ctrl[CTRL_MERGES], stream, &n)) return rc;
+    prev_n = n;
     if (n) {
       size_t bytes = tmp_bytes;
       GLIA_HIP_TRY(rocprim::radix_sort_pairs_desc(tmp, bytes, kseq, kseq2, vals, vals2, (size_t)n, 0, 64, stream));
@@ -339,7 +372,7 @@
     ws.nsort = n;
     std::string renv;
     ws.rebase_after = option("GLIA_HMT_REBASE", &renv) ? strtoull(renv.c_str(), nullptr, 10) : std::max<unsigned long long>(800000ull, (unsigned long long)n / 2ull);
-    ws.wch = 0;
+    ws.wch = 0; horizon_rule = "none";
     if (horizon_factor > 0.0 && n > 4096) {
       unsigned long long topkey = 0;
       GLIA_HIP_TRY(hipMemcpyAsync(&topkey, ksal2, sizeof(topkey), hipMemcpyDeviceToHost, stream));
@@ -349,6 +382,7 @@
         const double d = (double)std::max<long long>(0, prev_top_cell - top_cell);
         const double delta = std::max(horizon_factor * d * (double)ws.rebase_after / (double)(n_edges - prev_ne), (double)ws.wB / 512.0);
         ws.wch = (double)top_cell > delta ? (uint32_t)((double)top_cell - delta) : 0u;
+        if (ws.wch) horizon_rule = "descent";
       }
       prev_top_cell = top_cell; prev_ne = n_edges;
     }
@@ -397,7 +431,6 @@
   if (window) {
     if ((rc = entries.add(buf, &ws.fpool, st.pool_cap, stream))) return rc;
     if ((rc = edges.add(buf, &ws.er, st.Ecap, stream))) return rc;
-    if ((rc = edges.add(buf, &ws.ecat, st.Ecap, stream))) return rc;
   }
   else if ((rc = entries.add(buf, &st.pool, st.pool_cap, stream))) return rc;
   if ((rc = edges.add(buf, &st.e_u, st.Ecap, stream)) || (rc = edges.add(buf, &st.e_v, st.Ecap, stream)) ||
@@ -478,7 +511,10 @@
     if ((rc = base.init(buf, ws, st.pq.leaf_sal, E0, B, R, stream))) return rc;
     if (req.cond_n <= 0 && !batch_off) base.horizon_factor = option("GLIA_HMT_HORIZON", &o_txt) ? atof(o_txt.c_str()) : 0.5;
     base.from_lists = req.cond_n <= 0 && !batch_off;
-    if ((rc = base.rebaseline(ws, E0, ctrl, stream))) return rc;
+    if (option("GLIA_HMT_COLLECT_LANES", &o_txt)) { const int l = atoi(o_txt.c_str()); if (l == 16 || l == 64) base.force_lanes = l; }
+    base.check = option("GLIA_HMT_COLLECT_CHECK", &o_txt) && o_txt[0] == '1';
+    base.trace = option("GLIA_HMT_TRACE");
+    if ((rc = base.rebaseline(ws, E0, ctrl, stream, true))) return rc;
   } else if ((rc = pq_setup(buf, st.pq, stream))) return rc;
   GLIA_HIP_TRY(hipMemcpyAsync(st.ctrl, ctrl, sizeof(ctrl), hipMemcpyHostToDevice, stream));
   GLIA_HIP_TRY(hipEventRecord(ev.ev[1], stream));
@@ -503,7 +539,8 @@
     GLIA_HIP_TRY(hipGetLastError());
     GLIA_HIP_TRY(hipMemcpyAsync(ctrl, st.ctrl, sizeof(ctrl), hipMemcpyDeviceToHost, stream));
     GLIA_HIP_TRY(hipStreamSynchronize(stream));
-    if (trace) fprintf(stderr, "[trace] merge loop launch ended: status %llu, merges %llu of %u regions, edges %llu, list entries %llu, records rebuilt %llu\n", ctrl[CTRL_STATUS], ctrl[CTRL_MERGES], R, ctrl[CTRL_EDGES], ctrl[CTRL_ENTRIES], base.rebuilt_last);
+    if (trace) fprintf(stderr, "[trace] merge loop launch ended: status %llu, merges %llu of %u regions, edges %llu, list entries %llu, records rebuilt %llu; horizon cell %u of %u (%s)\n", ctrl[CTRL_STATUS], ctrl[CTRL_MERGES], R, ctrl[CTRL_EDGES], ctrl[CTRL_ENTRIES], base.rebuilt_last,
+                       window ? ws.wch : 0u, window ? ws.wB : 0u, window ? base.horizon_rule : "none");
     base.rebuilt_last = 0;
     if (ctrl[CTRL_STATUS] == ST_DONE) break;
     switch (ctrl[CTRL_STATUS]) {
@@ -525,7 +562,6 @@
         if (!window) return unhandled();
         entries.remove(&ws.fpool);
         edges.remove(&ws.er);
-        edges.remove(&ws.ecat);
         if ((rc = entries.add(buf, &st.pool, st.pool_cap, stream))) return rc;
         hipLaunchKernelGGL(fat_to_thin, dim3((unsigned)((ctrl[CTRL_ENTRIES] + 255) / 256)), dim3(256), 0, stream, ws.fpool, st.pool, ctrl[CTRL_ENTRIES]);
         if (base.from_lists) {
diff --git a/glia_amd/csrc/greedy_batch.hpp b/glia_amd/csrc/greedy_batch.hpp
--- a/glia_amd/csrc/greedy_batch.hpp
+++ b/glia_amd/csrc/greedy_batch.hpp
@@ -203,8 +203,8 @@
       double first;
       int second;
       if (mean_link(h0, f0.mean, (int)f0.n, h1, f1.mean, (int)f1.n, &first, &second)) bad = true;
-      const uint32_t offRs = f0.off, posRs = f0.pos, lenRs = f0.len;
-      if (h0 && h1) st.fpool[offRs + f1.pos].eid = kNone;
+      const uint32_t offRs = f0.off, posRs = entry_pos(f0), lenRs = f0.len;
+      if (h0 && h1) st.fpool[offRs + entry_pos(f1)].eid = kNone;
       const unsigned long long seq = update_seq(k, rs, r0, h0);
       const double sal = -first;
       const uint32_t cell = win_cell(sal, tau.smin, tau.scale, st.wB);
@@ -247,10 +247,14 @@
   uint32_t status = ST_RUN;
   win_enter(st, w, s, tid);
   if (tid == 0) { b.nkill = 0; b.kovf = 0; b.bad = 0; }
+#ifdef GLIA_HMT_PROFILE
+  if (tid < 8) g_reloadprof[tid] = 0;
+#endif
   b.bitmap[wave][lane] = 0;
   if (tid < kNW) { Key z; z.sal = -__builtin_inf(); z.seq = 0; z.arg = 0; b.part1[tid] = z; b.part2[tid] = z; }
   full_barrier();
   const double smin = st.wrange[0], scale = st.wrange[1];
+  asm volatile("" ::"v"(smin), "v"(scale));
   uint32_t pend_e = kNone, pend_old = kNone;
   constexpr uint32_t kTab = kMarkSlots / kNW;
   uint32_t* const tk = &s.mk[wave * kTab]; uint32_t* const t0 = &s.mv0[wave * kTab]; uint32_t* const t1 = &s.mv1[wave * kTab];
@@ -355,7 +359,7 @@
         }
         if (side1[p]) {
           t1[h[p]] = 1u;
-          sg_eid[h[p]] = fe[p].eid; sg_n[h[p]] = fe[p].n; sg_pos[h[p]] = fe[p].pos; sg_mean[h[p]] = fe[p].mean;
+          sg_eid[h[p]] = fe[p].eid; sg_n[h[p]] = fe[p].n; sg_pos[h[p]] = entry_pos(fe[p]); sg_mean[h[p]] = fe[p].mean;
         } else t0[h[p]] = 1u;
         atomicOr(&b.bitmap[wave][(fe[p].rs >> 5) & 63u], 1u << (fe[p].rs & 31u));
       }
@@ -451,7 +455,7 @@
         const bool h0 = !side1[p];
         const uint32_t rs = fe[p].rs;
         const uint32_t newE = (uint32_t)ne + my_ne + idx[p];
-        const uint32_t offRs = fe[p].off, posRs = fe[p].pos, lenRs = fe[p].len;
+        const uint32_t offRs = fe[p].off, posRs = entry_pos(fe[p]), lenRs = fe[p].len;
         if (both[p]) st.fpool[offRs + p_pos[p]].eid = kNone;
         const unsigned long long seq = update_seq(kk, rs, r0, h0);
         const double sal = -first[p];
@@ -484,6 +488,8 @@
                        atomicAdd(&g_edgeprof[2][0], 0ull), atomicAdd(&g_edgeprof[2][1], 0ull));
   if (tid == 0) printf("[batch profile] merges %llu: select %llu  compute %llu  validate %llu  commit %llu  scan %llu  loop-top %llu  reload %llu (cycles); rounds %llu candidates %llu committed %llu (cut by saliency %llu, by adjacency %llu) wide %llu\n",
                        k, bph[0], bph[1], bph[2], bph[3], bph[4], bph[5], bph[6], brounds, bmembers, bvalid, bcut_sal, bcut_dep, bwide);
+  if (tid == 0) printf("[batch profile] reload split (this launch; cycles of thread 0): sweeping cells %llu (%llu sweeps)  whole cells %llu  walks of split cells %llu (%llu cells); list nodes visited: live %llu dead %llu; horizon cell %u of %u\n",
+                       g_reloadprof[0], g_reloadprof[5], g_reloadprof[1], g_reloadprof[2], g_reloadprof[6], atomicAdd(&g_reloadprof[3], 0ull), atomicAdd(&g_reloadprof[4], 0ull), st.wch, st.wB);
   if (tid == 0) printf("[batch profile] scan phases (cumulative cycles, wave 0): loads %llu  compare %llu  top2 %llu  top2 with a tied best %llu  barrier %llu  calls %llu  tied second %llu  tied best %llu\n",
                        g_scanprof[0], g_scanprof[1], g_scanprof[2], g_scanprof[3], g_scanprof[4], g_scanprof[7], g_scanprof[5], g_scanprof[6]);
   if (tid == 0) printf("[batch profile] scan fill (cumulative; n <= 512, <= 1024, more): after reload/evict %llu %llu %llu  after narrow round %llu %llu %llu  after wide %llu %llu %llu\n",
diff --git a/glia_amd/csrc/greedy_window.hpp b/glia_amd/csrc/greedy_window.hpp
--- a/glia_amd/csrc/greedy_window.hpp
+++ b/glia_amd/csrc/greedy_window.hpp
@@ -24,7 +24,6 @@
   uint32_t wch;
   uint8_t* rdead;
   unsigned long long force_tree;
-  uint8_t* ecat;
 };
 constexpr uint32_t kWinCap = 1536;
 constexpr uint32_t kWinBudget = 768;
@@ -196,7 +195,22 @@
 }
 
 constexpr uint32_t kSelMax = 384;
+#ifdef GLIA_HMT_PROFILE
+__device__ unsigned long long g_reloadprof[8];
+#define RLD_T(i) do { if (tid == 0) { const unsigned long long tn_ = __builtin_readcyclecounter(); g_reloadprof[i] += tn_ - rt_; rt_ = tn_; } } while (0)
+#define RLD_MARK() do { if (tid == 0) rt_ = __builtin_readcyclecounter(); } while (0)
+#define RLD_NODE(alive) do { if (alive) ++rl_live; else ++rl_dead; } while (0)
+#define RLD_FLUSH() do { if (rl_live) atomicAdd(&g_reloadprof[3], (unsigned long long)rl_live); if (rl_dead) atomicAdd(&g_reloadprof[4], (unsigned long long)rl_dead); } while (0)
+#else
+#define RLD_T(i) do {} while (0)
+#define RLD_MARK() do {} while (0)
+#define RLD_NODE(alive) do {} while (0)
+#define RLD_FLUSH() do {} while (0)
+#endif
 __device__ __forceinline__ int win_reload(const WinState& st, WinShared& w, int tid, double* sel_sal, unsigned long long* sel_seq) {
+#ifdef GLIA_HMT_PROFILE
+  unsigned long long rt_ = 0; uint32_t rl_live = 0, rl_dead = 0;
+#endif
   full_barrier();
   if (tid == 0) { w.n = 0; w.need_tree = 0; }
   full_barrier();
@@ -204,6 +218,7 @@
   int result = 1;
   const uint32_t c_floor = st.wch < st.wB ? st.wch : 0u;
   while (c_hi > c_floor) {
+    RLD_MARK();
     const bool valid = (uint32_t)tid < c_hi - c_floor;
     const uint32_t c = valid ? c_hi - 1u - (uint32_t)tid : 0u;
     const uint32_t cn = valid ? ld_relaxed(&st.wcnt[c]) : 0u;
@@ -212,6 +227,10 @@
     const bool ok = valid && incl <= st.wbudget - loaded;
     const uint32_t m = (uint32_t)__syncthreads_count(ok ? 1 : 0);
     const uint32_t nvalid = c_hi - c_floor < (uint32_t)kGreedyThreads ? c_hi - c_floor : (uint32_t)kGreedyThreads;
+    RLD_T(0);
+#ifdef GLIA_HMT_PROFILE
+    if (tid == 0) g_reloadprof[5] += 1;
+#endif
     if (m != 0) {
       const uint32_t c_lo = c_hi - m;
       if ((uint32_t)tid == m - 1u) w.bcast = incl;
@@ -222,11 +241,12 @@
         uint32_t e = ld_relaxed(&st.whead[c]);
         if (e != kNone) {
           st_agent(&st.whead[c], kNone);
-          if (cn != 0) while (e != kNone) { const EdgeRec r = st.er[e]; win_take(st, w, e, r); e = r.next; }
+          if (cn != 0) while (e != kNone) { const EdgeRec r = st.er[e]; RLD_NODE(r.seq != 0); win_take(st, w, e, r); e = r.next; }
         }
         if (cn != 0) st_agent(&st.wcnt[c], 0u);
       }
       full_barrier();
+      RLD_T(1);
       loaded += w.bcast;
       c_hi = c_lo;
       if (loaded) result = 0;
@@ -238,10 +258,15 @@
         const uint32_t K = (room / 2u < kSelMax ? room / 2u : kSelMax) > 1u ? (room / 2u < kSelMax ? room / 2u : kSelMax) : 2u, RA = room > K ? room - K : 1u;
         const uint32_t seg_end = st.ige[cs];
         const uint32_t before = w.n;
+        RLD_MARK();
+#ifdef GLIA_HMT_PROFILE
+        if (tid == 0) g_reloadprof[6] += 1;
+#endif
         if (tid == 0) {
           uint32_t hn = 0, nlive = 0;
           for (uint32_t e = ld_relaxed(&st.whead[cs]); e != kNone;) {
             const EdgeRec r = st.er[e];
+            RLD_NODE(r.seq != 0);
             if (r.seq != 0) {
               ++nlive;
               if (hn < K) {
@@ -268,6 +293,7 @@
           }
           w.psal = nlive > K ? sel_sal[0] : -__builtin_inf(); w.pseq = nlive > K ? sel_seq[0] : 0ull;
         }
+        RLD_T(2);
         full_barrier();
         double tsal = w.psal; unsigned long long tseq = w.pseq;
         const uint32_t iA = seg_end > iptr ? (seg_end - iptr < RA ? seg_end : iptr + RA) : iptr;
@@ -288,8 +314,10 @@
         iptr += w.bcast;
         if (tid == 0) {
           uint32_t keep_head = kNone, keep_tail = kNone;
+          RLD_MARK();
           for (uint32_t e = ld_relaxed(&st.whead[cs]); e != kNone;) {
             const EdgeRec r = st.er[e];
+            RLD_NODE(r.seq != 0);
             if (r.seq != 0) {
               if (r.sal > tsal || (r.sal == tsal && r.seq > tseq)) win_take(st, w, e, r);
               else { if (keep_head == kNone) keep_head = e; else st.er[keep_tail].next = e; keep_tail = e; }
@@ -298,6 +326,7 @@
           }
           if (keep_tail != kNone) st.er[keep_tail].next = kNone;
           st_agent(&st.whead[cs], keep_head);
+          RLD_T(2);
         }
         full_barrier();
         const uint32_t moved = w.n - before;
@@ -310,6 +339,7 @@
         if (tid == 0) { if (moved) atomicSub(&st.wcnt[cs], moved); w.cthr = (int)cs; w.tsal = tsal; w.tseq = tseq; w.iptr = iptr; }
         if (moved || w.bcast) result = 0;
         full_barrier();
+        RLD_FLUSH();
         return result;
       }
       break;
@@ -319,6 +349,7 @@
   full_barrier();
   if (tid == 0 && result != 2) { w.cthr = (int)c_hi - 1; w.tsal = __builtin_inf(); w.tseq = ~0ull; w.iptr = iptr; }
   full_barrier();
+  RLD_FLUSH();
   if (result == 1 && c_floor != 0u) result = 3;
   return result;
 }
@@ -373,8 +404,7 @@
 template <bool BATCH>
 __device__ __forceinline__ void store_new_edge(const WinState& st, uint32_t newE, uint32_t rs, uint32_t r2, uint32_t posRs, uint32_t idx, double first, int second,
                                                double sal, unsigned long long seq, uint32_t offRs, uint32_t lenRs, uint32_t r2off, uint32_t lenR2, uint32_t cell) {
-  if (BATCH && cell < st.wch) st.ecat[newE] = (uint8_t)((uint32_t)(seq >> 30) & 3u);
-  else {
+  if (!(BATCH && cell < st.wch)) {
     uint4* pq4 = reinterpret_cast<uint4*>(&st.er[newE]);
     pq4[0] = make_uint4(rs, r2, posRs, idx);
     const unsigned long long mb = (unsigned long long)__double_as_longlong(first);
@@ -385,7 +415,7 @@
   }
   FatEntry a; a.eid = newE; a.rs = r2; a.n = (uint32_t)second; a.pos = idx; a.off = r2off; a.len = lenR2; a.mean = first;
   st.fpool[offRs + posRs] = a;
-  FatEntry b; b.eid = newE; b.rs = rs; b.n = (uint32_t)second; b.pos = posRs; b.off = offRs; b.len = lenRs; b.mean = first;
+  FatEntry b; b.eid = newE; b.rs = rs; b.n = (uint32_t)second; b.pos = pack_pos(posRs, (uint32_t)(seq >> 30) & 3u); b.off = offRs; b.len = lenRs; b.mean = first;
   st.fpool[r2off + idx] = b;
 }
 template <bool BATCH>
@@ -421,7 +451,7 @@
 __device__ __forceinline__ void win_complete_r2(const WinState& st, int tid, uint32_t ne, uint32_t r2off, uint32_t newcount, double smin, double scale) {
   for (uint32_t j = tid; j < newcount; j += kGreedyThreads) {
     const FatEntry fb = st.fpool[r2off + j];
-    st.fpool[fb.off + fb.pos].len = newcount;
+    st.fpool[fb.off + entry_pos(fb)].len = newcount;
     if (!BATCH || win_cell(-fb.mean, smin, scale, st.wB) >= st.wch) st.er[ne + j].hv.y = newcount;
     st.mark0[fb.rs] = 0; st.mark1[fb.rs] = 0;
   }
@@ -566,8 +596,8 @@
       double first;
       int second;
       if (mean_link(h0, f0.mean, (int)f0.n, h1, f1.mean, (int)f1.n, &first, &second)) bad = true;
-      const uint32_t offRs = f0.off, posRs = f0.pos, lenRs = f0.len;
-      if (h0 && h1) st.fpool[offRs + f1.pos].eid = kNone;
+      const uint32_t offRs = f0.off, posRs = entry_pos(f0), lenRs = f0.len;
+      if (h0 && h1) st.fpool[offRs + entry_pos(f1)].eid = kNone;
       const unsigned long long seq = update_seq(k, rs, r0, h0);
       const double sal = -first;
       const uint32_t cell = win_cell(sal, tau.smin, tau.scale, st.wB);
```

After: 322,700. No clear change (-0.1%).
